# amazon-science/gan-control

Hardware: AMD Instinct MI355X
Metric: images/sec G+D step FFHQ-1024 (higher is better)
Workload: dtype bf16x3; 1 GPU; FFHQ 1024x1024 full G+D train step (D step, G step, lazy R1 every 16 and path-length every 4, Adam, EMA), 4 images/GPU, fp32 storage, conv arithmetic bf16x3; global_batch=4, parallelism=dp1

## Files before the change

### gan-control_amd/csrc/bias_act.hip

```cpp
#include "common.h"

namespace {

__device__ __forceinline__ float lrelu_gain(float v, float slope, float gain) {
    return (v > 0.f ? v : v * slope) * gain;
}

template <bool VEC, bool NOISE>
__global__ __launch_bounds__(256) void bias_act_plane_kernel(
    const float* __restrict__ x, const float* __restrict__ bias, const float* __restrict__ noise,
    const float* __restrict__ noise_w, float* __restrict__ y, int channels, int64_t inner, float slope, float gain) {
    const int plane = blockIdx.y;
    const int c = plane % channels, b = plane / channels;
    const float bv = bias ? bias[c] : 0.f;
    const float nw = NOISE ? noise_w[0] : 0.f;
    const float* xp = x + (size_t)plane * inner;
    float* yp = y + (size_t)plane * inner;
    const float* np = NOISE ? noise + (size_t)b * inner : nullptr;
    if (VEC) {
        const int64_t n4 = inner >> 2;
        for (int64_t i = (int64_t)blockIdx.x * 256 + threadIdx.x; i < n4; i += (int64_t)gridDim.x * 256) {
            const gc::f32x4_t xv = gc::stream_load4(xp + 4 * i);
            float4 v = make_float4(xv.x, xv.y, xv.z, xv.w);
            if (NOISE) {
                const float4 nz = reinterpret_cast<const float4*>(np)[i];
                v.x = fmaf(nw, nz.x, v.x); v.y = fmaf(nw, nz.y, v.y); v.z = fmaf(nw, nz.z, v.z); v.w = fmaf(nw, nz.w, v.w);
            }
            v.x = lrelu_gain(v.x + bv, slope, gain); v.y = lrelu_gain(v.y + bv, slope, gain);
            v.z = lrelu_gain(v.z + bv, slope, gain); v.w = lrelu_gain(v.w + bv, slope, gain);
            gc::stream_store4(yp + 4 * i, v.x, v.y, v.z, v.w);
        }
    } else {
        for (int64_t i = (int64_t)blockIdx.x * 256 + threadIdx.x; i < inner; i += (int64_t)gridDim.x * 256) {
            float v = xp[i];
            if (NOISE) v = fmaf(nw, np[i], v);
            yp[i] = lrelu_gain(v + bv, slope, gain);
        }
    }
}

template <bool NOISE>
__global__ __launch_bounds__(256) void bias_act_flat_kernel(
    const float* __restrict__ x, const float* __restrict__ bias, const float* __restrict__ noise,
    const float* __restrict__ noise_w, float* __restrict__ y, int channels, int inner, int64_t total, float slope, float gain) {
    const float nw = NOISE ? noise_w[0] : 0.f;
    for (int64_t i = (int64_t)blockIdx.x * 256 + threadIdx.x; i < total; i += (int64_t)gridDim.x * 256) {
        const int64_t plane = i / inner;
        const int p = (int)(i - plane * inner);
        const int c = (int)(plane % channels);
        float v = x[i];
        if (NOISE) v = fmaf(nw, noise[(plane / channels) * inner + p], v);
        y[i] = lrelu_gain(v + (bias ? bias[c] : 0.f), slope, gain);
    }
}

#ifndef GC_BWD_RUN
#define GC_BWD_RUN 1024
#endif
constexpr int BWD_RUN = GC_BWD_RUN;
template <bool VEC>
__global__ __launch_bounds__(256) void bias_act_bwd_kernel(
    const float* __restrict__ dy, const float* __restrict__ yref, float* __restrict__ dx, int64_t count, float pos, float neg) {
    if (VEC) {
        const int64_t n4 = count >> 2;
        const int64_t lo = (int64_t)blockIdx.x * BWD_RUN, hi = min(n4, lo + BWD_RUN);
        for (int64_t i = lo + threadIdx.x; i < hi; i += 256) {
            const gc::f32x4_t g = gc::stream_load4(dy + 4 * i);
            const gc::f32x4_t r = gc::stream_load4(yref + 4 * i);
            float4 o;
            o.x = g.x * (r.x > 0.f ? pos : neg); o.y = g.y * (r.y > 0.f ? pos : neg);
            o.z = g.z * (r.z > 0.f ? pos : neg); o.w = g.w * (r.w > 0.f ? pos : neg);
            gc::stream_store4(dx + 4 * i, o.x, o.y, o.z, o.w);
        }
        if (blockIdx.x == 0)
            for (int64_t i = (n4 << 2) + threadIdx.x; i < count; i += 256) dx[i] = dy[i] * (yref[i] > 0.f ? pos : neg);
    } else {
        const int64_t lo = (int64_t)blockIdx.x * (4 * BWD_RUN), hi = min(count, lo + 4 * BWD_RUN);
        for (int64_t i = lo + threadIdx.x; i < hi; i += 256) dx[i] = dy[i] * (yref[i] > 0.f ? pos : neg);
    }
}

__device__ __forceinline__ float wave_sum(float v) {
#pragma unroll
    for (int off = 32; off > 0; off >>= 1) v += __shfl_down(v, off, 64);
    return v;
}

__device__ __forceinline__ float block_sum(float v, float* lds) {
    v = wave_sum(v);
    const int lane = threadIdx.x & 63, wave = threadIdx.x >> 6;
    if (lane == 0) lds[wave] = v;
    __syncthreads();
    float r = 0.f;
    if (threadIdx.x == 0) r = lds[0] + lds[1] + lds[2] + lds[3];
    __syncthreads();
    return r;
}

template <bool NOISE, bool SELF>
__global__ __launch_bounds__(256) void bias_act_bwd_reduce_kernel(
    const float* __restrict__ dy, const float* __restrict__ yref, const float* __restrict__ noise, const float* __restrict__ bias,
    const float* __restrict__ noise_w, float* __restrict__ dx, float* __restrict__ psum, float* __restrict__ pdot, float* __restrict__ pself,
    int channels, int64_t inner, int chunks, int64_t chunk_len, float pos, float neg) {
    __shared__ float lds[4];
    const int plane = blockIdx.x / chunks, j = blockIdx.x - plane * chunks;
    const int b = plane / channels, c = plane % channels;
    const size_t base = (size_t)plane * inner;
    const float* np = NOISE ? noise + (size_t)b * inner : nullptr;
    const float bv = (SELF && bias) ? bias[c] : 0.f, nw = (SELF && NOISE) ? noise_w[0] : 0.f;
    const float ipos = 1.f / pos, ineg = 1.f / neg;
    const int64_t lo = (int64_t)j * chunk_len, hi = min(inner, lo + chunk_len);
    float s = 0.f, d = 0.f, q = 0.f;
    auto one = [&](float yv, float dyv, float nz) {
        const float g = dyv * (yv > 0.f ? pos : neg);
        s += g;
        if (NOISE) d = fmaf(g, nz, d);
        if (SELF) q = fmaf(g, yv * (yv > 0.f ? ipos : ineg) - bv - nw * nz, q);
        return g;
    };
    typedef float f4u __attribute__((ext_vector_type(4), aligned(4)));
    const int64_t n4 = (hi - lo) >> 2;
    for (int64_t v = threadIdx.x; v < n4; v += 256) {
        const int64_t i = lo + 4 * v;
        const f4u y4 = gc::stream_load4u(yref + base + i), g4 = gc::stream_load4u(dy + base + i);
        f4u z4 = {0.f, 0.f, 0.f, 0.f};
        if (NOISE) z4 = *reinterpret_cast<const f4u*>(np + i);
        const f4u o4 = {one(y4.x, g4.x, z4.x), one(y4.y, g4.y, z4.y), one(y4.z, g4.z, z4.z), one(y4.w, g4.w, z4.w)};
        gc::stream_store4u(dx + base + i, o4.x, o4.y, o4.z, o4.w);
    }
    for (int64_t i = lo + 4 * n4 + threadIdx.x; i < hi; i += 256)
        dx[base + i] = one(yref[base + i], dy[base + i], NOISE ? np[i] : 0.f);
    const float rs = block_sum(s, lds);
    if (threadIdx.x == 0) psum[(size_t)plane * chunks + j] = rs;
    if (NOISE) {
        const float rd = block_sum(d, lds);
        if (threadIdx.x == 0) pdot[(size_t)plane * chunks + j] = rd;
    }
    if (SELF) {
        const float rq = block_sum(q, lds);
        if (threadIdx.x == 0) pself[(size_t)plane * chunks + j] = rq;
    }
}

__global__ __launch_bounds__(256) void bias_act_bwd_reduce_adjoint_kernel(
    const float* __restrict__ ggx, const float* __restrict__ cs, const float* __restrict__ cd, const float* __restrict__ cw,
    const float* __restrict__ yref, const float* __restrict__ dx, const float* __restrict__ noise, const float* __restrict__ bias,
    const float* __restrict__ noise_w, float* __restrict__ g_dy, float* __restrict__ g_yref, float* __restrict__ pgb, float* __restrict__ pgn,
    int channels, int64_t inner, int chunks, int64_t chunk_len, float pos, float neg) {
    __shared__ float lds[4];
    const int plane = blockIdx.x / chunks, j = blockIdx.x - plane * chunks;
    const int b = plane / channels, c = plane % channels;
    const size_t base = (size_t)plane * inner, pj = (size_t)plane * chunks + j;
    const float* np = noise ? noise + (size_t)b * inner : nullptr;
    const float bv = bias ? bias[c] : 0.f, nw = (noise && noise_w) ? noise_w[0] : 0.f;
    const float ipos = 1.f / pos, ineg = 1.f / neg;
    const float vs = cs ? cs[pj] : 0.f, vd = (cd && noise) ? cd[pj] : 0.f, vw = cw ? cw[pj] : 0.f;
    const int64_t lo = (int64_t)j * chunk_len, hi = min(inner, lo + chunk_len);
    float sb = 0.f, sn = 0.f;
    typedef float f4u __attribute__((ext_vector_type(4), aligned(4)));
    auto one = [&](float yv, float gg, float gxv, float nz, float* gyref) {
        const bool up = yv > 0.f;
        const float xpre = yv * (up ? ipos : ineg) - bv - nw * nz;
        const float total = gg + vs + vd * nz + vw * xpre;
        const float wg = vw * gxv;
        sb += wg;
        sn = fmaf(wg, nz, sn);
        *gyref = wg * (up ? ipos : ineg);
        return total * (up ? pos : neg);
    };
    const int64_t n4 = (hi - lo) >> 2;
    for (int64_t v = threadIdx.x; v < n4; v += 256) {
        const int64_t i = lo + 4 * v;
        const f4u y4 = *reinterpret_cast<const f4u*>(yref + base + i);
        f4u g4 = {0.f, 0.f, 0.f, 0.f}, x4 = g4, z4 = g4;
        if (ggx) g4 = *reinterpret_cast<const f4u*>(ggx + base + i);
        if (cw) x4 = *reinterpret_cast<const f4u*>(dx + base + i);
        if (np) z4 = *reinterpret_cast<const f4u*>(np + i);
        float r0, r1, r2, r3;
        const f4u o4 = {one(y4.x, g4.x, x4.x, z4.x, &r0), one(y4.y, g4.y, x4.y, z4.y, &r1), one(y4.z, g4.z, x4.z, z4.z, &r2), one(y4.w, g4.w, x4.w, z4.w, &r3)};
        gc::stream_store4u(g_dy + base + i, o4.x, o4.y, o4.z, o4.w);
        if (g_yref) gc::stream_store4u(g_yref + base + i, r0, r1, r2, r3);
    }
    for (int64_t i = lo + 4 * n4 + threadIdx.x; i < hi; i += 256) {
        float r;
        g_dy[base + i] = one(yref[base + i], ggx ? ggx[base + i] : 0.f, cw ? dx[base + i] : 0.f, np ? np[i] : 0.f, &r);
        if (g_yref) g_yref[base + i] = r;
    }
    if (pgb) {
        const float rb = block_sum(sb, lds);
        if (threadIdx.x == 0) pgb[pj] = rb;
    }
    if (pgn) {
        const float rn = block_sum(sn, lds);
        if (threadIdx.x == 0) pgn[pj] = rn;
    }
}

__global__ __launch_bounds__(256) void plane_dot_kernel(const float* __restrict__ a, const float* __restrict__ b, float* __restrict__ partial,
                                                        int64_t inner, int chunks, int64_t chunk_len) {
    __shared__ float lds[4];
    const int plane = blockIdx.x / chunks, j = blockIdx.x - plane * chunks;
    const size_t base = (size_t)plane * inner;
    const int64_t lo = (int64_t)j * chunk_len, hi = min(inner, lo + chunk_len);
    float acc = 0.f;
    typedef float f4u __attribute__((ext_vector_type(4), aligned(4)));
    const int64_t n4 = (hi - lo) >> 2;
    for (int64_t v = threadIdx.x; v < n4; v += 256) {
        const int64_t i = lo + 4 * v;
        const f4u a4 = gc::stream_load4u(a + base + i), b4 = gc::stream_load4u(b + base + i);
        acc = fmaf(a4.x, b4.x, acc); acc = fmaf(a4.y, b4.y, acc); acc = fmaf(a4.z, b4.z, acc); acc = fmaf(a4.w, b4.w, acc);
    }
    for (int64_t i = lo + 4 * n4 + threadIdx.x; i < hi; i += 256) acc = fmaf(a[base + i], b[base + i], acc);
    const float r = block_sum(acc, lds);
    if (threadIdx.x == 0) partial[(size_t)plane * chunks + j] = r;
}

__global__ __launch_bounds__(256) void rows_sum_div_kernel(const float* __restrict__ partial, const float* __restrict__ den, float* __restrict__ out,
                                                           int rows, int chunks) {
    const int r = blockIdx.x * 256 + threadIdx.x;
    if (r >= rows) return;
    float acc = 0.f;
    for (int j = 0; j < chunks; ++j) acc += partial[(size_t)r * chunks + j];
    if (den) { const float d = den[r]; acc = acc / (d == 0.f ? 1.f : d); }
    out[r] = acc;
}

__global__ __launch_bounds__(256) void plane_dot_pitched_kernel(const float* __restrict__ a, const float* __restrict__ b, float* __restrict__ partial,
                                                                int rows, int width, int a_pitch, int b_pitch, int chunks, int rpc) {
    __shared__ float lds[4];
    const int plane = blockIdx.x / chunks, j = blockIdx.x - plane * chunks;
    const float* ap = a + (size_t)plane * rows * a_pitch;
    const float* bp = b + (size_t)plane * rows * b_pitch;
    const int r0 = j * rpc, r1 = min(rows, r0 + rpc);
    typedef float f4u __attribute__((ext_vector_type(4), aligned(4)));
    const int lane = threadIdx.x & 63, wave = threadIdx.x >> 6;
    const int w4 = width >> 2;
    float acc0 = 0.f, acc1 = 0.f;
    for (int r = r0 + wave; r < r1; r += 4) {
        const float* ar = ap + (size_t)r * a_pitch;
        const float* br = bp + (size_t)r * b_pitch;
        int v = lane;
        for (; v + 64 < w4; v += 128) {
            const f4u a0 = *reinterpret_cast<const f4u*>(ar + 4 * v), b0 = *reinterpret_cast<const f4u*>(br + 4 * v);
            const f4u a1 = *reinterpret_cast<const f4u*>(ar + 4 * (v + 64)), b1 = *reinterpret_cast<const f4u*>(br + 4 * (v + 64));
            acc0 = fmaf(a0.x, b0.x, acc0); acc0 = fmaf(a0.y, b0.y, acc0); acc0 = fmaf(a0.z, b0.z, acc0); acc0 = fmaf(a0.w, b0.w, acc0);
            acc1 = fmaf(a1.x, b1.x, acc1); acc1 = fmaf(a1.y, b1.y, acc1); acc1 = fmaf(a1.z, b1.z, acc1); acc1 = fmaf(a1.w, b1.w, acc1);
        }
        for (; v < w4; v += 64) {
            const f4u a0 = *reinterpret_cast<const f4u*>(ar + 4 * v), b0 = *reinterpret_cast<const f4u*>(br + 4 * v);
            acc0 = fmaf(a0.x, b0.x, acc0); acc0 = fmaf(a0.y, b0.y, acc0); acc0 = fmaf(a0.z, b0.z, acc0); acc0 = fmaf(a0.w, b0.w, acc0);
        }
        for (int c = 4 * w4 + lane; c < width; c += 64) acc1 = fmaf(ar[c], br[c], acc1);
    }
    const float s = block_sum(acc0 + acc1, lds);
    if (threadIdx.x == 0) partial[(size_t)plane * chunks + j] = s;
}

__global__ __launch_bounds__(256) void channel_sum_stage1(const float* __restrict__ x, float* __restrict__ partial,
                                                          int batch, int channels, int64_t inner, int chunks, int64_t chunk_len) {
    __shared__ float lds[4];
    const int plane = blockIdx.x / chunks, j = blockIdx.x - plane * chunks;
    const int c = plane % channels, b = plane / channels;
    const float* xp = x + (size_t)plane * inner;
    const int64_t lo = (int64_t)j * chunk_len, hi = min(inner, lo + chunk_len);
    float acc = 0.f;
    if (((inner | lo | hi) & 3) == 0 && (reinterpret_cast<uintptr_t>(xp) & 15) == 0) {
        const float4* x4 = reinterpret_cast<const float4*>(xp);
        float a0 = 0.f, a1 = 0.f, a2 = 0.f, a3 = 0.f;
#pragma unroll 4
        for (int64_t i = lo / 4 + threadIdx.x; i < hi / 4; i += 256) {
            const gc::f32x4_t v = gc::stream_load4(reinterpret_cast<const float*>(x4 + i));
            a0 += v.x; a1 += v.y; a2 += v.z; a3 += v.w;
        }
        acc = (a0 + a1) + (a2 + a3);
    } else {
        for (int64_t i = lo + threadIdx.x; i < hi; i += 256) acc += xp[i];
    }
    const float r = block_sum(acc, lds);
    if (threadIdx.x == 0) partial[((size_t)c * batch + b) * chunks + j] = r;
}

__global__ __launch_bounds__(256) void channel_sum_stage2(const float* __restrict__ partial, float* __restrict__ out, int n) {
    __shared__ float lds[4];
    const int c = blockIdx.x;
    float acc = 0.f;
    for (int i = threadIdx.x; i < n; i += 256) acc += partial[(size_t)c * n + i];
    const float r = block_sum(acc, lds);
    if (threadIdx.x == 0) out[c] = r;
}

inline void channel_sum_plan(int64_t inner, int* chunks, int64_t* chunk_len) {
#ifndef GC_SUM_LEN
#define GC_SUM_LEN 16384
#endif
    int64_t len = GC_SUM_LEN;
    int n = (int)gc::ceil_div64(inner, len);
    if (n < 1) n = 1;
    *chunks = n;
    *chunk_len = len;
}

inline bool aligned16(const void* p) { return (reinterpret_cast<uintptr_t>(p) & 15) == 0; }

}

extern "C" int gc_bias_act_f32(const float* x, const float* bias, const float* noise, const float* noise_w,
                               float* y, int batch, int channels, int64_t inner, float slope, float gain, gc_stream_t stream) {
    if (!x || !y) return gc::fail(GC_ERR_BAD_ARG, "gc_bias_act_f32: null pointer");
    if ((noise == nullptr) != (noise_w == nullptr)) return gc::fail(GC_ERR_BAD_ARG, "gc_bias_act_f32: noise and noise_w must both be set or both be null");
    if (batch < 0 || channels <= 0 || inner <= 0) return gc::fail(GC_ERR_BAD_ARG, "gc_bias_act_f32: bad extents");
    if (batch == 0) return GC_OK;
    hipStream_t s = (hipStream_t)stream;
    const int64_t planes = (int64_t)batch * channels;
    if (inner >= 1024 && planes <= 65535) {
        const bool vec = (inner % 4 == 0) && aligned16(x) && aligned16(y) && (!noise || aligned16(noise));
        const int64_t work = vec ? inner / 4 : inner;
        dim3 grid((unsigned)std::min<int64_t>(gc::ceil_div64(work, 256 * 4), 1024), (unsigned)planes);
#define GC_LAUNCH(V, N) hipLaunchKernelGGL((bias_act_plane_kernel<V, N>), grid, dim3(256), 0, s, x, bias, noise, noise_w, y, channels, inner, slope, gain)
        if (vec) { if (noise) GC_LAUNCH(true, true); else GC_LAUNCH(true, false); }
        else     { if (noise) GC_LAUNCH(false, true); else GC_LAUNCH(false, false); }
#undef GC_LAUNCH
        return gc::check_launch("gc_bias_act_f32(plane)");
    }
    if (inner > INT32_MAX) return gc::fail(GC_ERR_UNSUPPORTED, "gc_bias_act_f32: inner too large for the flat path");
    const int64_t total = planes * inner;
    const int blocks = (int)std::min<int64_t>(gc::ceil_div64(total, 256), 4096);
    if (noise)
        hipLaunchKernelGGL(bias_act_flat_kernel<true>, dim3(blocks), dim3(256), 0, s, x, bias, noise, noise_w, y, channels, (int)inner, total, slope, gain);
    else
        hipLaunchKernelGGL(bias_act_flat_kernel<false>, dim3(blocks), dim3(256), 0, s, x, bias, noise, noise_w, y, channels, (int)inner, total, slope, gain);
    return gc::check_launch("gc_bias_act_f32(flat)");
}

extern "C" int gc_bias_act_bwd_f32(const float* dy, const float* y_ref, float* dx, int64_t count,
                                   float slope, float gain, gc_stream_t stream) {
    if (!dy || !y_ref || !dx) return gc::fail(GC_ERR_BAD_ARG, "gc_bias_act_bwd_f32: null pointer");
    if (count < 0) return gc::fail(GC_ERR_BAD_ARG, "gc_bias_act_bwd_f32: negative count");
    if (count == 0) return GC_OK;
    hipStream_t s = (hipStream_t)stream;
    const bool vec = aligned16(dy) && aligned16(y_ref) && aligned16(dx);
    const int64_t nblocks = gc::ceil_div64(count, 4 * (int64_t)BWD_RUN);
    if (nblocks > INT32_MAX) return gc::fail(GC_ERR_UNSUPPORTED, "gc_bias_act_bwd_f32: more than 2^31 blocks");
    const int blocks = (int)nblocks;
    if (vec)
        hipLaunchKernelGGL(bias_act_bwd_kernel<true>, dim3(blocks), dim3(256), 0, s, dy, y_ref, dx, count, gain, gain * slope);
    else
        hipLaunchKernelGGL(bias_act_bwd_kernel<false>, dim3(blocks), dim3(256), 0, s, dy, y_ref, dx, count, gain, gain * slope);
    return gc::check_launch("gc_bias_act_bwd_f32");
}

extern "C" size_t gc_channel_sum_workspace(int batch, int channels, int64_t inner) {
    if (batch <= 0 || channels <= 0 || inner <= 0) return 0;
    int chunks; int64_t len;
    channel_sum_plan(inner, &chunks, &len);
    return (size_t)batch * channels * chunks * sizeof(float);
}

extern "C" int gc_channel_sum_f32(const float* x, float* out, int batch, int channels, int64_t inner,
                                  void* workspace, size_t workspace_bytes, gc_stream_t stream) {
    if (!x || !out) return gc::fail(GC_ERR_BAD_ARG, "gc_channel_sum_f32: null pointer");
    if (batch <= 0 || channels <= 0 || inner <= 0) return gc::fail(GC_ERR_BAD_ARG, "gc_channel_sum_f32: bad extents");
    if ((int64_t)batch * channels * gc_bias_act_bwd_chunks(inner) > INT32_MAX) return gc::fail(GC_ERR_UNSUPPORTED, "gc_channel_sum_f32: more than 2^31 blocks");
    const size_t need = gc_channel_sum_workspace(batch, channels, inner);
    if (!workspace || workspace_bytes < need) return gc::fail(GC_ERR_WORKSPACE, "gc_channel_sum_f32: workspace %zu < %zu bytes", workspace_bytes, need);
    hipStream_t s = (hipStream_t)stream;
    int chunks; int64_t len;
    channel_sum_plan(inner, &chunks, &len);
    float* partial = static_cast<float*>(workspace);
    hipLaunchKernelGGL(channel_sum_stage1, dim3((unsigned)chunks * (unsigned)(batch * channels)), dim3(256), 0, s, x, partial, batch, channels, inner, chunks, len);
    int rc = gc::check_launch("gc_channel_sum_f32(stage1)");
    if (rc) return rc;
    hipLaunchKernelGGL(channel_sum_stage2, dim3(channels), dim3(256), 0, s, partial, out, batch * chunks);
    return gc::check_launch("gc_channel_sum_f32(stage2)");
}

extern "C" int gc_bias_act_bwd_chunks(int64_t inner) {
    if (inner <= 0) return 0;
    int chunks; int64_t len;
    channel_sum_plan(inner, &chunks, &len);
    return chunks;
}

extern "C" int gc_bias_act_bwd_reduce_self_f32(const float* dy, const float* y_ref, const float* noise, const float* bias, const float* noise_w,
                                               float* dx, float* psum, float* pdot, float* pself, int batch, int channels, int64_t inner,
                                               float slope, float gain, gc_stream_t stream) {
    if (!dy || !y_ref || !dx || !psum) return gc::fail(GC_ERR_BAD_ARG, "gc_bias_act_bwd_reduce_f32: null pointer");
    if ((noise == nullptr) != (pdot == nullptr)) return gc::fail(GC_ERR_BAD_ARG, "gc_bias_act_bwd_reduce_f32: noise and pdot go together");
    if (pself && noise && !noise_w) return gc::fail(GC_ERR_BAD_ARG, "gc_bias_act_bwd_reduce_f32: pself with noise needs noise_w");
    if (pself && (slope == 0.f || gain == 0.f)) return gc::fail(GC_ERR_UNSUPPORTED, "gc_bias_act_bwd_reduce_f32: pself needs an invertible activation (slope, gain != 0)");
    if (batch <= 0 || channels <= 0 || inner <= 0) return gc::fail(GC_ERR_BAD_ARG, "gc_bias_act_bwd_reduce_f32: bad extents");
    hipStream_t s = (hipStream_t)stream;
    int chunks; int64_t len;
    channel_sum_plan(inner, &chunks, &len);
    if ((int64_t)batch * channels * chunks > INT32_MAX) return gc::fail(GC_ERR_UNSUPPORTED, "gc_bias_act_bwd_reduce_f32: more than 2^31 blocks");
    dim3 grid((unsigned)chunks * (unsigned)(batch * channels));
#define GC_LAUNCH(N, S) hipLaunchKernelGGL((bias_act_bwd_reduce_kernel<N, S>), grid, dim3(256), 0, s, dy, y_ref, noise, bias, noise_w, dx, psum, pdot, pself, \
                                           channels, inner, chunks, len, gain, gain * slope)
    if (noise) { if (pself) GC_LAUNCH(true, true); else GC_LAUNCH(true, false); }
    else       { if (pself) GC_LAUNCH(false, true); else GC_LAUNCH(false, false); }
#undef GC_LAUNCH
    return gc::check_launch("gc_bias_act_bwd_reduce_f32");
}

extern "C" int gc_bias_act_bwd_reduce_adjoint_f32(const float* ggx, const float* cs, const float* cd, const float* cw, const float* y_ref, const float* dx,
                                                  const float* noise, const float* bias, const float* noise_w, float* g_dy, float* g_yref, float* pgb, float* pgn,
                                                  int batch, int channels, int64_t inner, float slope, float gain, gc_stream_t stream) {
    if (!y_ref || !g_dy) return gc::fail(GC_ERR_BAD_ARG, "gc_bias_act_bwd_reduce_adjoint_f32: null pointer");
    if (cw && !dx) return gc::fail(GC_ERR_BAD_ARG, "gc_bias_act_bwd_reduce_adjoint_f32: cw needs dx");
    if (cw && noise && !noise_w) return gc::fail(GC_ERR_BAD_ARG, "gc_bias_act_bwd_reduce_adjoint_f32: cw with noise needs noise_w");
    if (cd && !noise) return gc::fail(GC_ERR_BAD_ARG, "gc_bias_act_bwd_reduce_adjoint_f32: cd needs noise");
    if (slope == 0.f || gain == 0.f) return gc::fail(GC_ERR_UNSUPPORTED, "gc_bias_act_bwd_reduce_adjoint_f32: needs an invertible activation (slope, gain != 0)");
    if (batch <= 0 || channels <= 0 || inner <= 0) return gc::fail(GC_ERR_BAD_ARG, "gc_bias_act_bwd_reduce_adjoint_f32: bad extents");
    int chunks; int64_t len;
    channel_sum_plan(inner, &chunks, &len);
    if ((int64_t)batch * channels * chunks > INT32_MAX) return gc::fail(GC_ERR_UNSUPPORTED, "gc_bias_act_bwd_reduce_adjoint_f32: more than 2^31 blocks");
    hipLaunchKernelGGL(bias_act_bwd_reduce_adjoint_kernel, dim3((unsigned)chunks * (unsigned)(batch * channels)), dim3(256), 0, (hipStream_t)stream, ggx, cs, cd, cw, y_ref, dx,
                       noise, bias, noise_w, g_dy, g_yref, pgb, pgn, channels, inner, chunks, len, gain, gain * slope);
    return gc::check_launch("gc_bias_act_bwd_reduce_adjoint_f32");
}

extern "C" int gc_bias_act_bwd_reduce_f32(const float* dy, const float* y_ref, const float* noise, float* dx,
                                          float* psum, float* pdot, int batch, int channels, int64_t inner,
                                          float slope, float gain, gc_stream_t stream) {
    return gc_bias_act_bwd_reduce_self_f32(dy, y_ref, noise, nullptr, nullptr, dx, psum, pdot, nullptr, batch, channels, inner, slope, gain, stream);
}

static void plane_dot_pitched_plan(int rows, int* chunks, int* rpc) {
    *rpc = rows <= 64 ? rows : 32;
    *chunks = (rows + *rpc - 1) / *rpc;
}

extern "C" int gc_plane_dot_pitched_chunks(int rows) {
    if (rows <= 0) return 0;
    int chunks, rpc;
    plane_dot_pitched_plan(rows, &chunks, &rpc);
    return chunks;
}

extern "C" int gc_plane_dot_pitched_f32(const float* a, const float* b, float* partial, int planes, int rows, int width, int a_pitch, int b_pitch,
                                        gc_stream_t stream) {
    if (!a || !b || !partial) return gc::fail(GC_ERR_BAD_ARG, "gc_plane_dot_pitched_f32: null pointer");
    if (planes <= 0 || rows <= 0 || width <= 0 || a_pitch < width || b_pitch < width) return gc::fail(GC_ERR_BAD_ARG, "gc_plane_dot_pitched_f32: bad extents");
    int chunks, rpc;
    plane_dot_pitched_plan(rows, &chunks, &rpc);
    if ((int64_t)planes * chunks > INT32_MAX) return gc::fail(GC_ERR_UNSUPPORTED, "gc_plane_dot_pitched_f32: more than 2^31 blocks");
    hipLaunchKernelGGL(plane_dot_pitched_kernel, dim3((unsigned)planes * (unsigned)chunks), dim3(256), 0, (hipStream_t)stream,
                       a, b, partial, rows, width, a_pitch, b_pitch, chunks, rpc);
    return gc::check_launch("gc_plane_dot_pitched_f32");
}

extern "C" int gc_rows_sum_div_f32(const float* partial, const float* den, float* out, int rows, int chunks, gc_stream_t stream) {
    if (!partial || !out) return gc::fail(GC_ERR_BAD_ARG, "gc_rows_sum_div_f32: null pointer");
    if (rows <= 0 || chunks <= 0) return gc::fail(GC_ERR_BAD_ARG, "gc_rows_sum_div_f32: bad extents");
    hipLaunchKernelGGL(rows_sum_div_kernel, dim3((unsigned)((rows + 255) / 256)), dim3(256), 0, (hipStream_t)stream, partial, den, out, rows, chunks);
    return gc::check_launch("gc_rows_sum_div_f32");
}

extern "C" int gc_plane_dot_f32(const float* a, const float* b, float* partial, int planes, int64_t inner, gc_stream_t stream) {
    if (!a || !b || !partial) return gc::fail(GC_ERR_BAD_ARG, "gc_plane_dot_f32: null pointer");
    if (planes <= 0 || inner <= 0) return gc::fail(GC_ERR_BAD_ARG, "gc_plane_dot_f32: bad extents");
    int chunks; int64_t len;
    channel_sum_plan(inner, &chunks, &len);
    if ((int64_t)planes * chunks > INT32_MAX) return gc::fail(GC_ERR_UNSUPPORTED, "gc_plane_dot_f32: more than 2^31 blocks");
    hipLaunchKernelGGL(plane_dot_kernel, dim3((unsigned)chunks * (unsigned)planes), dim3(256), 0, (hipStream_t)stream, a, b, partial, inner, chunks, len);
    return gc::check_launch("gc_plane_dot_f32");
}
```

### gan-control_amd/csrc/upfirdn2d.hip

```cpp
#include "common.h"

namespace {

constexpr int TH = 32, TW = 128;
constexpr int PH = TH + 3, PW = TW + 3;
constexpr int PITCH = 132;

struct FirEpilogue {
    const float* bias; const float* noise; const float* noise_w;
    float slope, gain; int channels;
    const float* mask_ref; float mpos, mneg;
    const float* pro_ref; const float* pro_noise; float* pro_psum; float* pro_pdot; float ppos, pneg;
};

#ifndef GC_FIR_NT
#define GC_FIR_NT 1
#endif

#ifndef GC_FIR_OCC
#define GC_FIR_OCC 0
#endif
#if GC_FIR_OCC > 0
#define GC_FIR_BOUNDS __launch_bounds__(256, GC_FIR_OCC)
#else
#define GC_FIR_BOUNDS __launch_bounds__(256)
#endif
template <bool VEC, int EPI, bool PRO = false>
__global__ GC_FIR_BOUNDS void fir44_tile_kernel(
    const float* __restrict__ x, const float* __restrict__ taps, float* __restrict__ y,
    int in_h, int in_w, int out_h, int out_w, int pad_x0, int pad_y0, int flip, FirEpilogue ep, int in_pitch, int out_pitch) {
    __shared__ __attribute__((aligned(16))) float patch[PH * PITCH];
    const int tid = threadIdx.x;
    const int ox0 = blockIdx.x * TW;
    const size_t plane = blockIdx.z;
    const float* xp = x + plane * (size_t)in_h * in_pitch;
    float* yp = y + plane * (size_t)out_h * out_pitch;

    float T[4][4];
#pragma unroll
    for (int a = 0; a < 4; ++a)
#pragma unroll
        for (int b = 0; b < 4; ++b) T[a][b] = flip ? taps[(3 - a) * 4 + (3 - b)] : taps[a * 4 + b];

    const int ix0 = ox0 - pad_x0;
    constexpr int GPR = PITCH / 4;
    constexpr int NLD = (PH * GPR + 255) / 256;
    typedef float f4u __attribute__((ext_vector_type(4), aligned(4)));
    float4 stage[NLD];
    auto ld4 = [&](const float* rowp, int ix, int width) {
        float4 v = make_float4(0.f, 0.f, 0.f, 0.f);
        const float* src = rowp + ix;
        if (ix >= 0 && ix + 3 < width) {
            const f4u t = *reinterpret_cast<const f4u*>(src);
            v = make_float4(t.x, t.y, t.z, t.w);
        } else {
            if (ix >= 0 && ix < width) v.x = src[0];
            if (ix + 1 >= 0 && ix + 1 < width) v.y = src[1];
            if (ix + 2 >= 0 && ix + 2 < width) v.z = src[2];
            if (ix + 3 >= 0 && ix + 3 < width) v.w = src[3];
        }
        return v;
    };
    static_assert(!PRO || GC_FIR_NT == 1, "the prologue sums are written once per workgroup");
    float ps = 0.f, pd = 0.f;
    const float* refp = PRO ? ep.pro_ref + plane * (size_t)in_h * in_w : nullptr;
    const float* nzp = (PRO && ep.pro_noise) ? ep.pro_noise + (plane / ep.channels) * (size_t)in_h * in_w : nullptr;
    auto fetch = [&](int oy0) {
        const int iy0 = oy0 - pad_y0;
#pragma unroll
        for (int j = 0; j < NLD; ++j) {
            const int idx = tid + 256 * j;
            const int r = idx / GPR, c = (idx - r * GPR) * 4;
            const int iy = iy0 + r, ix = ix0 + c;
            float4 v = make_float4(0.f, 0.f, 0.f, 0.f);
            if (idx < PH * GPR && iy >= 0 && iy < in_h) {
                v = ld4(xp + (size_t)iy * in_pitch, ix, in_w);
                if (PRO) {
                    const float4 m = ld4(refp + (size_t)iy * in_w, ix, in_w);
                    v.x *= m.x > 0.f ? ep.ppos : ep.pneg; v.y *= m.y > 0.f ? ep.ppos : ep.pneg;
                    v.z *= m.z > 0.f ? ep.ppos : ep.pneg; v.w *= m.w > 0.f ? ep.ppos : ep.pneg;
                    if ((r < TH || blockIdx.y == gridDim.y - 1) && (c < TW || blockIdx.x == gridDim.x - 1)) {
                        ps += (v.x + v.y) + (v.z + v.w);
                        if (nzp) {
                            const float4 z = ld4(nzp + (size_t)iy * in_w, ix, in_w);
                            pd += (v.x * z.x + v.y * z.y) + (v.z * z.z + v.w * z.w);
                        }
                    }
                }
            }
            stage[j] = v;
        }
    };
    auto commit = [&]() {
#pragma unroll
        for (int j = 0; j < NLD; ++j) {
            const int idx = tid + 256 * j;
            if (idx < PH * GPR) *reinterpret_cast<float4*>(&patch[idx * 4]) = stage[j];
        }
    };

    const int cg = tid & 31, rg = tid >> 5;
    const int ox = ox0 + cg * 4;
    const int ty0 = blockIdx.y * GC_FIR_NT;
    const int tiles_y = (out_h + TH - 1) / TH;
    const int nt = min(GC_FIR_NT, tiles_y - ty0);
    fetch(ty0 * TH);
    __shared__ float red[8];
    if (PRO) {
#pragma unroll
        for (int off = 32; off > 0; off >>= 1) { ps += __shfl_xor(ps, off, 64); pd += __shfl_xor(pd, off, 64); }
        if ((tid & 63) == 0) { red[(tid >> 6) * 2] = ps; red[(tid >> 6) * 2 + 1] = pd; }
    }
    commit();
    __syncthreads();
    if (PRO && tid == 0) {
        const size_t slot = plane * ((size_t)gridDim.x * gridDim.y) + (size_t)blockIdx.y * gridDim.x + blockIdx.x;
        ep.pro_psum[slot] = (red[0] + red[2]) + (red[4] + red[6]);
        if (ep.pro_pdot) ep.pro_pdot[slot] = (red[1] + red[3]) + (red[5] + red[7]);
    }
    for (int t = 0; t < nt; ++t) {
        const int oy0 = (ty0 + t) * TH;
        const bool more = t + 1 < nt;
        if (more) fetch(oy0 + TH);

        float acc[4][4];
#pragma unroll
        for (int r = 0; r < 4; ++r)
#pragma unroll
            for (int j = 0; j < 4; ++j) acc[r][j] = 0.f;

#pragma unroll
        for (int i = 0; i < 7; ++i) {
            const float* row = &patch[(rg * 4 + i) * PITCH + cg * 4];
            const float4 lo = *reinterpret_cast<const float4*>(row);
            const float v4 = row[4], v5 = row[5], v6 = row[6];
            const float v[7] = {lo.x, lo.y, lo.z, lo.w, v4, v5, v6};
#pragma unroll
            for (int r = 0; r < 4; ++r) {
                const int a = i - r;
                if (a < 0 || a > 3) continue;
#pragma unroll
                for (int j = 0; j < 4; ++j)
#pragma unroll
                    for (int b = 0; b < 4; ++b) acc[r][j] = fmaf(T[a][b], v[j + b], acc[r][j]);
            }
        }

        if (EPI == 2) {
            const float* ref = ep.mask_ref + plane * (size_t)out_h * out_w;
            float m[4][4];
            const bool vec_ref = VEC && (out_w & 3) == 0 && ((reinterpret_cast<uintptr_t>(ref) & 15) == 0);
#pragma unroll
            for (int r = 0; r < 4; ++r) {
                const int oy = oy0 + rg * 4 + r;
                if (vec_ref && oy < out_h && ox + 3 < out_w) {
                    const float4 t = *reinterpret_cast<const float4*>(ref + (size_t)oy * out_w + ox);
                    m[r][0] = t.x; m[r][1] = t.y; m[r][2] = t.z; m[r][3] = t.w;
                } else {
#pragma unroll
                    for (int j = 0; j < 4; ++j) m[r][j] = (oy < out_h && ox + j < out_w) ? ref[(size_t)oy * out_w + ox + j] : 0.f;
                }
            }
#pragma unroll
            for (int r = 0; r < 4; ++r)
#pragma unroll
                for (int j = 0; j < 4; ++j) acc[r][j] *= m[r][j] > 0.f ? ep.mpos : ep.mneg;
        }
        if (EPI == 1) {
            const int c = (int)(plane % ep.channels);
            const size_t b = plane / ep.channels;
            const float bv = ep.bias ? ep.bias[c] : 0.f, nw = ep.noise ? ep.noise_w[0] : 0.f;
            float nz[4][4];
#pragma unroll
            for (int r = 0; r < 4; ++r)
#pragma unroll
                for (int j = 0; j < 4; ++j) {
                    const int oy = oy0 + rg * 4 + r;
                    nz[r][j] = (ep.noise && oy < out_h && ox + j < out_w) ? ep.noise[(b * out_h + oy) * out_w + ox + j] : 0.f;
                }
#pragma unroll
            for (int r = 0; r < 4; ++r)
#pragma unroll
                for (int j = 0; j < 4; ++j) {
                    const float v = fmaf(nw, nz[r][j], acc[r][j]) + bv;
                    acc[r][j] = (v > 0.f ? v : v * ep.slope) * ep.gain;
                }
        }
        if (more) {
            __syncthreads();
            commit();
            __syncthreads();
        }
#pragma unroll
        for (int r = 0; r < 4; ++r) {
            const int oy = oy0 + rg * 4 + r;
            if (oy >= out_h) break;
            float* dst = yp + (size_t)oy * out_pitch + ox;
            if (VEC) {
                if (ox + 3 < out_w) gc::stream_store4(dst, acc[r][0], acc[r][1], acc[r][2], acc[r][3]);
                else {
#pragma unroll
                    for (int j = 0; j < 4; ++j)
                        if (ox + j < out_w) dst[j] = acc[r][j];
                }
            } else if (ox + 3 < out_w) {
                gc::stream_store4u(dst, acc[r][0], acc[r][1], acc[r][2], acc[r][3]);
            } else {
#pragma unroll
                for (int j = 0; j < 4; ++j)
                    if (ox + j < out_w) dst[j] = acc[r][j];
            }
        }
    }
}


constexpr int D_TH = 16, D_TW = 128;
constexpr int D_PH = 2 * D_TH + 2, D_PW = 2 * D_TW + 2, D_PITCH = 260;

template <bool VEC>
__global__ __launch_bounds__(256) void fir44_down2_kernel(
    const float* __restrict__ x, const float* __restrict__ taps, float* __restrict__ y,
    int in_h, int in_w, int out_h, int out_w, int pad_x0, int pad_y0, int flip) {
    __shared__ __attribute__((aligned(16))) float patch[D_PH * D_PITCH];
    const int tid = threadIdx.x;
    const int ox0 = blockIdx.x * D_TW, oy0 = blockIdx.y * D_TH;
    const size_t plane = blockIdx.z;
    const float* xp = x + plane * (size_t)in_h * in_w;
    float* yp = y + plane * (size_t)out_h * out_w;

    float T[4][4];
#pragma unroll
    for (int a = 0; a < 4; ++a)
#pragma unroll
        for (int b = 0; b < 4; ++b) T[a][b] = flip ? taps[(3 - a) * 4 + (3 - b)] : taps[a * 4 + b];

    const int iy0 = 2 * oy0 - pad_y0, ix0 = 2 * ox0 - pad_x0;
    constexpr int GPR = D_PITCH / 4;
    constexpr int NLD = (D_PH * GPR + 255) / 256;
    typedef float f4u __attribute__((ext_vector_type(4), aligned(4)));
    float4 stage[NLD];
#pragma unroll
    for (int j = 0; j < NLD; ++j) {
        const int idx = tid + 256 * j;
        const int r = idx / GPR, c = (idx - r * GPR) * 4;
        const int iy = iy0 + r, ix = ix0 + c;
        float4 v = make_float4(0.f, 0.f, 0.f, 0.f);
        if (idx < D_PH * GPR && iy >= 0 && iy < in_h) {
            const float* src = xp + (size_t)iy * in_w + ix;
            if (ix >= 0 && ix + 3 < in_w) {
                const f4u t = *reinterpret_cast<const f4u*>(src);
                v = make_float4(t.x, t.y, t.z, t.w);
            } else {
                if (ix >= 0 && ix < in_w) v.x = src[0];
                if (ix + 1 >= 0 && ix + 1 < in_w) v.y = src[1];
                if (ix + 2 >= 0 && ix + 2 < in_w) v.z = src[2];
                if (ix + 3 >= 0 && ix + 3 < in_w) v.w = src[3];
            }
        }
        stage[j] = v;
    }
#pragma unroll
    for (int j = 0; j < NLD; ++j) {
        const int idx = tid + 256 * j;
        if (idx < D_PH * GPR) *reinterpret_cast<float4*>(&patch[idx * 4]) = stage[j];
    }
    __syncthreads();

    const int cg = tid & 31, rg = tid >> 5;
    float acc[2][4];
#pragma unroll
    for (int r = 0; r < 2; ++r)
#pragma unroll
        for (int j = 0; j < 4; ++j) acc[r][j] = 0.f;
#pragma unroll
    for (int i = 0; i < 6; ++i) {
        const float* row = &patch[(rg * 4 + i) * D_PITCH + cg * 8];
        const float4 q0 = *reinterpret_cast<const float4*>(row), q1 = *reinterpret_cast<const float4*>(row + 4);
        const float2 q2 = *reinterpret_cast<const float2*>(row + 8);
        const float v[10] = {q0.x, q0.y, q0.z, q0.w, q1.x, q1.y, q1.z, q1.w, q2.x, q2.y};
#pragma unroll
        for (int r = 0; r < 2; ++r) {
            const int a = i - 2 * r;
            if (a < 0 || a > 3) continue;
#pragma unroll
            for (int j = 0; j < 4; ++j)
#pragma unroll
                for (int b = 0; b < 4; ++b) acc[r][j] = fmaf(T[a][b], v[2 * j + b], acc[r][j]);
        }
    }
    const int ox = ox0 + cg * 4;
#pragma unroll
    for (int r = 0; r < 2; ++r) {
        const int oy = oy0 + rg * 2 + r;
        if (oy >= out_h) break;
        float* dst = yp + (size_t)oy * out_w + ox;
        if (VEC) {
            if (ox + 3 < out_w) gc::stream_store4(dst, acc[r][0], acc[r][1], acc[r][2], acc[r][3]);
        } else if (ox + 3 < out_w) {
            gc::stream_store4u(dst, acc[r][0], acc[r][1], acc[r][2], acc[r][3]);
        } else {
#pragma unroll
            for (int j = 0; j < 4; ++j)
                if (ox + j < out_w) dst[j] = acc[r][j];
        }
    }
}

constexpr int U_TH = 32, U_TW = 128;
constexpr int U_PH = U_TH / 2 + 3, U_PW = U_TW / 2 + 3, U_PITCH = 68;

template <int EY, int EX, bool VEC>
__global__ __launch_bounds__(256) void fir44_up2_kernel(
    const float* __restrict__ x, const float* __restrict__ taps, float* __restrict__ y,
    int in_h, int in_w, int out_h, int out_w, int pad_x0, int pad_y0, int flip) {
    __shared__ __attribute__((aligned(16))) float patch[U_PH * U_PITCH];
    const int tid = threadIdx.x;
    const int ox0 = blockIdx.x * U_TW, oy0 = blockIdx.y * U_TH;
    const size_t plane = blockIdx.z;
    const float* xp = x + plane * (size_t)in_h * in_w;
    float* yp = y + plane * (size_t)out_h * out_w;

    float T[4][4];
#pragma unroll
    for (int a = 0; a < 4; ++a)
#pragma unroll
        for (int b = 0; b < 4; ++b) T[a][b] = flip ? taps[(3 - a) * 4 + (3 - b)] : taps[a * 4 + b];

    const int iy0 = (oy0 - pad_y0) >> 1, ix0 = (ox0 - pad_x0) >> 1;
    constexpr int NLD = (U_PH * U_PITCH + 255) / 256;
    float stage[NLD];
#pragma unroll
    for (int j = 0; j < NLD; ++j) {
        const int idx = tid + 256 * j;
        const int r = idx / U_PITCH, c = idx - r * U_PITCH;
        const int iy = iy0 + r, ix = ix0 + c;
        float v = 0.f;
        if (idx < U_PH * U_PITCH && c < U_PW && iy >= 0 && iy < in_h && ix >= 0 && ix < in_w) v = xp[(size_t)iy * in_w + ix];
        stage[j] = v;
    }
#pragma unroll
    for (int j = 0; j < NLD; ++j) {
        const int idx = tid + 256 * j;
        if (idx < U_PH * U_PITCH) patch[idx] = stage[j];
    }
    __syncthreads();

    const int cg = tid & 31, rg = tid >> 5;
    float w[4][4];
#pragma unroll
    for (int i = 0; i < 4; ++i) {
        const float* row = &patch[(rg * 2 + i) * U_PITCH + cg * 2];
        const float2 lo = *reinterpret_cast<const float2*>(row), hi = *reinterpret_cast<const float2*>(row + 2);
        w[i][0] = lo.x; w[i][1] = lo.y; w[i][2] = hi.x; w[i][3] = hi.y;
    }
    const int ox = ox0 + cg * 4;
#pragma unroll
    for (int r = 0; r < 4; ++r) {
        const int a0 = (EY + r) & 1, qy = (EY + r + a0) >> 1;
        float o[4];
#pragma unroll
        for (int j = 0; j < 4; ++j) {
            const int b0 = (EX + j) & 1, qx = (EX + j + b0) >> 1;
            float s = 0.f;
#pragma unroll
            for (int i = 0; i < 2; ++i)
#pragma unroll
                for (int jj = 0; jj < 2; ++jj) s = fmaf(T[a0 + 2 * i][b0 + 2 * jj], w[qy + i][qx + jj], s);
            o[j] = s;
        }
        const int oy = oy0 + rg * 4 + r;
        if (oy < out_h) {
            float* dst = yp + (size_t)oy * out_w + ox;
            if (VEC) {
                if (ox + 3 < out_w) gc::stream_store4(dst, o[0], o[1], o[2], o[3]);
            } else if (ox + 3 < out_w) {
                gc::stream_store4u(dst, o[0], o[1], o[2], o[3]);
            } else {
#pragma unroll
                for (int j = 0; j < 4; ++j)
                    if (ox + j < out_w) dst[j] = o[j];
            }
        }
    }
}

constexpr int SMALL_LDS_FLOATS = 4096, SMALL_PLANE_MAX = 36 * 36;

__global__ __launch_bounds__(256) void fir44_small_kernel(
    const float* __restrict__ x, const float* __restrict__ taps, float* __restrict__ y,
    int planes, int in_h, int in_w, int out_h, int out_w, int pad_x0, int pad_y0, int flip, int ppw) {
    __shared__ float L[SMALL_LDS_FLOATS];
    __shared__ float T[16];
    const int tid = threadIdx.x;
    if (tid < 16) T[tid] = flip ? taps[15 - tid] : taps[tid];
    const int lh = out_h + 3, lw = out_w + 3, lp = lh * lw;
    const int p0 = blockIdx.x * ppw, np = min(ppw, planes - p0);
    const float* xb = x + (size_t)p0 * in_h * in_w;
    for (int i = tid; i < np * lp; i += 256) {
        const int pl = i / lp, rem = i - pl * lp;
        const int r = rem / lw, c = rem - r * lw;
        const int iy = r - pad_y0, ix = c - pad_x0;
        L[i] = (iy >= 0 && iy < in_h && ix >= 0 && ix < in_w) ? xb[((size_t)pl * in_h + iy) * in_w + ix] : 0.f;
    }
    __syncthreads();
    const int op = out_h * out_w;
    float* yb = y + (size_t)p0 * op;
    for (int i = tid; i < np * op; i += 256) {
        const int pl = i / op, rem = i - pl * op;
        const int oy = rem / out_w, ox = rem - oy * out_w;
        const float* l = L + pl * lp + oy * lw + ox;
        float acc = 0.f;
#pragma unroll
        for (int a = 0; a < 4; ++a)
#pragma unroll
            for (int b = 0; b < 4; ++b) acc = fmaf(T[a * 4 + b], l[a * lw + b], acc);
        yb[i] = acc;
    }
}

constexpr int MAX_GENERIC_TAPS = 1024;

__global__ __launch_bounds__(256) void generic_kernel(
    const float* __restrict__ x, const float* __restrict__ taps, float* __restrict__ y,
    int planes, int in_h, int in_w, int out_h, int out_w, int kh, int kw,
    int up_x, int up_y, int down_x, int down_y, int pad_x0, int pad_y0, int flip) {
    __shared__ float T[MAX_GENERIC_TAPS];
    const int nt = kh * kw;
    for (int i = threadIdx.x; i < nt; i += 256) T[i] = flip ? taps[nt - 1 - i] : taps[i];
    __syncthreads();
    const size_t total = (size_t)planes * out_h * out_w;
    for (size_t idx = (size_t)blockIdx.x * 256 + threadIdx.x; idx < total; idx += (size_t)gridDim.x * 256) {
        const int ox = (int)(idx % out_w);
        const size_t t = idx / out_w;
        const int oy = (int)(t % out_h);
        const size_t plane = t / out_h;
        const float* xp = x + plane * (size_t)in_h * in_w;
        const int uy0 = oy * down_y - pad_y0, ux0 = ox * down_x - pad_x0;
        const int a0 = gc::pos_mod(-uy0, up_y), b0 = gc::pos_mod(-ux0, up_x);
        float acc = 0.f;
        for (int a = a0; a < kh; a += up_y) {
            const int uy = uy0 + a;
            if (uy < 0) continue;
            const int iy = uy / up_y;
            if (iy >= in_h) break;
            for (int b = b0; b < kw; b += up_x) {
                const int ux = ux0 + b;
                if (ux < 0) continue;
                const int ix = ux / up_x;
                if (ix >= in_w) break;
                acc = fmaf(T[a * kw + b], xp[(size_t)iy * in_w + ix], acc);
            }
        }
        y[idx] = acc;
    }
}

template <int K, int UP, int DOWN>
struct FirKCfg {
    static constexpr int TW = 64, TH = 16;
    static constexpr int PW = ((TW - 1) * DOWN + K - 1) / UP + 2, PH = ((TH - 1) * DOWN + K - 1) / UP + 2;
    static constexpr int PITCH = PW | 1;
};

template <int K, int UP, int DOWN>
__global__ __launch_bounds__(256) void firK_tile_kernel(
    const float* __restrict__ x, const float* __restrict__ taps, float* __restrict__ y,
    int in_h, int in_w, int out_h, int out_w, int pad_x0, int pad_y0, int flip) {
    using C = FirKCfg<K, UP, DOWN>;
    __shared__ float patch[C::PH * C::PITCH];
    __shared__ float T[K * K];
    const int tid = threadIdx.x;
    const int ox0 = blockIdx.x * C::TW, oy0 = blockIdx.y * C::TH;
    const size_t plane = blockIdx.z;
    const float* xp = x + plane * (size_t)in_h * in_w;
    float* yp = y + plane * (size_t)out_h * out_w;
    for (int i = tid; i < K * K; i += 256) T[i] = flip ? taps[K * K - 1 - i] : taps[i];
    const int ux_base = ox0 * DOWN - pad_x0, uy_base = oy0 * DOWN - pad_y0;
    const int ixb = gc::floor_div(ux_base, UP), iyb = gc::floor_div(uy_base, UP);
    for (int i = tid; i < C::PH * C::PW; i += 256) {
        const int r = i / C::PW, c = i - r * C::PW;
        const int iy = iyb + r, ix = ixb + c;
        patch[r * C::PITCH + c] = (iy >= 0 && iy < in_h && ix >= 0 && ix < in_w) ? xp[(size_t)iy * in_w + ix] : 0.f;
    }
    __syncthreads();
    const int ty = tid >> 4, tx = (tid & 15) * 4;
    const int oy = oy0 + ty;
    if (oy >= out_h) return;
    const int uy0 = oy * DOWN - pad_y0;
    const int a0 = gc::pos_mod(-uy0, UP);
    float acc[4] = {0.f, 0.f, 0.f, 0.f};
    int b0[4], cx[4];
#pragma unroll
    for (int i = 0; i < 4; ++i) {
        const int ux0 = (ox0 + tx + i) * DOWN - pad_x0;
        b0[i] = gc::pos_mod(-ux0, UP);
        cx[i] = (ux0 + b0[i] - ixb * UP) / UP;
    }
    constexpr int NA = (K + UP - 1) / UP;
#pragma unroll 2
    for (int aa = 0; aa < NA; ++aa) {
        const int a = a0 + aa * UP;
        if (a >= K) break;
        const float* prow = patch + ((uy0 + a - iyb * UP) / UP) * C::PITCH;
        const float* trow = T + a * K;
#pragma unroll
        for (int bb = 0; bb < NA; ++bb) {
#pragma unroll
            for (int i = 0; i < 4; ++i) {
                const int b = b0[i] + bb * UP;
                if (UP == 1 || b < K) acc[i] = fmaf(trow[b], prow[cx[i] + bb], acc[i]);
            }
        }
    }
#pragma unroll
    for (int i = 0; i < 4; ++i)
        if (ox0 + tx + i < out_w) yp[(size_t)oy * out_w + ox0 + tx + i] = acc[i];
}

template <int K>
int launch_firK(const float* x, const float* taps, float* y, int planes, int in_h, int in_w, int out_h, int out_w,
                int up, int down, int pad_x0, int pad_y0, int flip, hipStream_t s) {
    using C = FirKCfg<K, 1, 1>;
    dim3 grid(gc::ceil_div(out_w, C::TW), gc::ceil_div(out_h, C::TH), planes);
    if (up == 2 && down == 1)
        hipLaunchKernelGGL((firK_tile_kernel<K, 2, 1>), grid, dim3(256), 0, s, x, taps, y, in_h, in_w, out_h, out_w, pad_x0, pad_y0, flip);
    else if (up == 1 && down == 2)
        hipLaunchKernelGGL((firK_tile_kernel<K, 1, 2>), grid, dim3(256), 0, s, x, taps, y, in_h, in_w, out_h, out_w, pad_x0, pad_y0, flip);
    else
        hipLaunchKernelGGL((firK_tile_kernel<K, 1, 1>), grid, dim3(256), 0, s, x, taps, y, in_h, in_w, out_h, out_w, pad_x0, pad_y0, flip);
    return gc::check_launch("gc_upfirdn2d_f32(firK_tile)");
}

}

namespace {

int upfirdn2d_impl(const float* x, const float* taps, float* y,
                   int planes, int in_h, int in_w, int out_h, int out_w,
                   int kh, int kw, int up_x, int up_y, int down_x, int down_y,
                   int pad_x0, int pad_y0, int flip_taps, const FirEpilogue* ep, gc_stream_t stream, int in_pitch = 0, int out_pitch = 0) {
    if (in_pitch == 0) in_pitch = in_w;
    if (out_pitch == 0) out_pitch = out_w;
    if (out_pitch < out_w) return gc::fail(GC_ERR_BAD_ARG, "gc_upfirdn2d_f32: output pitch %d < width %d", out_pitch, out_w);
    if (in_pitch < in_w) return gc::fail(GC_ERR_BAD_ARG, "gc_upfirdn2d_f32: input pitch %d < width %d", in_pitch, in_w);
    if (!x || !taps || !y) return gc::fail(GC_ERR_BAD_ARG, "gc_upfirdn2d_f32: null pointer");
    if (planes < 0 || in_h <= 0 || in_w <= 0 || kh <= 0 || kw <= 0 || up_x <= 0 || up_y <= 0 || down_x <= 0 || down_y <= 0)
        return gc::fail(GC_ERR_BAD_ARG, "gc_upfirdn2d_f32: non-positive extent or factor");
    if (out_h <= 0 || out_w <= 0) return gc::fail(GC_ERR_BAD_ARG, "gc_upfirdn2d_f32: empty output (%d x %d)", out_h, out_w);
    if (planes == 0) return GC_OK;
    hipStream_t s = (hipStream_t)stream;
    const bool fast = up_x == 1 && up_y == 1 && down_x == 1 && down_y == 1 && kh == 4 && kw == 4 &&
                      out_w >= 64 && out_h >= 16 && planes <= 65535;
    if (ep && !fast) return gc::fail(GC_ERR_UNSUPPORTED, "gc_upfirdn2d_act_f32: the fused epilogue needs the 4x4, up = down = 1 tile kernel (planes >= 64 x 16)");
    if ((in_pitch != in_w || out_pitch != out_w) && !fast) return gc::fail(GC_ERR_UNSUPPORTED, "gc_upfirdn2d_pitched_f32: a pitched input needs the 4x4, up = down = 1 tile kernel (planes >= 64 x 16)");
    if (fast) {
        dim3 grid(gc::ceil_div(out_w, TW), gc::ceil_div(gc::ceil_div(out_h, TH), GC_FIR_NT), planes);
        const bool vec = (out_pitch % 4 == 0) && ((reinterpret_cast<uintptr_t>(y) & 15) == 0);
        const FirEpilogue none{nullptr, nullptr, nullptr, 1.f, 1.f, 1, nullptr, 1.f, 1.f, nullptr, nullptr, nullptr, nullptr, 1.f, 1.f};
        if (ep && ep->pro_ref) {
            if (in_pitch != in_w) return gc::fail(GC_ERR_UNSUPPORTED, "gc_upfirdn2d_actbwd_f32: the gradient must have dense rows");
            if (vec) hipLaunchKernelGGL((fir44_tile_kernel<true, 0, true>), grid, dim3(256), 0, s, x, taps, y, in_h, in_w, out_h, out_w, pad_x0, pad_y0, flip_taps, *ep, in_pitch, out_pitch);
            else     hipLaunchKernelGGL((fir44_tile_kernel<false, 0, true>), grid, dim3(256), 0, s, x, taps, y, in_h, in_w, out_h, out_w, pad_x0, pad_y0, flip_taps, *ep, in_pitch, out_pitch);
            return gc::check_launch("gc_upfirdn2d_actbwd_f32");
        }
#define GC_FIR(V, E) hipLaunchKernelGGL((fir44_tile_kernel<V, E>), grid, dim3(256), 0, s, x, taps, y, in_h, in_w, out_h, out_w, pad_x0, pad_y0, flip_taps, ep ? *ep : none, in_pitch, out_pitch)
        if (ep && ep->mask_ref) { if (vec) GC_FIR(true, 2); else GC_FIR(false, 2); }
        else if (ep) { if (vec) GC_FIR(true, 1); else GC_FIR(false, 1); }
        else    { if (vec) GC_FIR(true, 0); else GC_FIR(false, 0); }
#undef GC_FIR
        return gc::check_launch("gc_upfirdn2d_f32(fir44_tile)");
    }
    if (kh == 4 && kw == 4 && up_x == 1 && up_y == 1 && down_x == 1 && down_y == 1 && (out_h + 3) * (out_w + 3) <= SMALL_PLANE_MAX) {
        const int ppw = std::max(1, std::min(SMALL_LDS_FLOATS / ((out_h + 3) * (out_w + 3)), 1024 / std::max(1, out_h * out_w) + 1));
        hipLaunchKernelGGL(fir44_small_kernel, dim3(gc::ceil_div(planes, ppw)), dim3(256), 0, s, x, taps, y, planes, in_h, in_w, out_h, out_w,
                           pad_x0, pad_y0, flip_taps, ppw);
        return gc::check_launch("gc_upfirdn2d_f32(fir44_small)");
    }
    const bool square44 = kh == 4 && kw == 4 && up_x == up_y && down_x == down_y && planes <= 65535 && out_w >= 32 && out_h >= 8;
    const bool vec_ok = (out_w % 4 == 0) && ((reinterpret_cast<uintptr_t>(y) & 15) == 0);
    if (square44 && up_x == 1 && down_x == 2) {
        dim3 grid(gc::ceil_div(out_w, D_TW), gc::ceil_div(out_h, D_TH), planes);
        if (vec_ok)
            hipLaunchKernelGGL(fir44_down2_kernel<true>, grid, dim3(256), 0, s, x, taps, y, in_h, in_w, out_h, out_w, pad_x0, pad_y0, flip_taps);
        else
            hipLaunchKernelGGL(fir44_down2_kernel<false>, grid, dim3(256), 0, s, x, taps, y, in_h, in_w, out_h, out_w, pad_x0, pad_y0, flip_taps);
        return gc::check_launch("gc_upfirdn2d_f32(fir44_down2)");
    }
    if (square44 && up_x == 2 && down_x == 1) {
        dim3 grid(gc::ceil_div(out_w, U_TW), gc::ceil_div(out_h, U_TH), planes);
        const int ey = pad_y0 & 1, ex = pad_x0 & 1;
#define GC_UP2(EY, EX)                                                                                                             \
        if (ey == EY && ex == EX) {                                                                                                \
            if (vec_ok) hipLaunchKernelGGL((fir44_up2_kernel<EY, EX, true>), grid, dim3(256), 0, s, x, taps, y, in_h, in_w, out_h, out_w, pad_x0, pad_y0, flip_taps); \
            else hipLaunchKernelGGL((fir44_up2_kernel<EY, EX, false>), grid, dim3(256), 0, s, x, taps, y, in_h, in_w, out_h, out_w, pad_x0, pad_y0, flip_taps);       \
        }
        GC_UP2(0, 0) GC_UP2(0, 1) GC_UP2(1, 0) GC_UP2(1, 1)
#undef GC_UP2
        return gc::check_launch("gc_upfirdn2d_f32(fir44_up2)");
    }
    if (kh == 12 && kw == 12 && up_x == up_y && down_x == down_y && up_x * down_x <= 2 && planes <= 65535 && out_w >= 32 && out_h >= 8)
        return launch_firK<12>(x, taps, y, planes, in_h, in_w, out_h, out_w, up_x, down_x, pad_x0, pad_y0, flip_taps, s);
    if (kh * kw > MAX_GENERIC_TAPS) return gc::fail(GC_ERR_UNSUPPORTED, "gc_upfirdn2d_f32: %d x %d taps exceed %d", kh, kw, MAX_GENERIC_TAPS);
    const size_t total = (size_t)planes * out_h * out_w;
    const int blocks = (int)std::min<size_t>((total + 255) / 256, 256 * 16);
    hipLaunchKernelGGL(generic_kernel, dim3(blocks), dim3(256), 0, s, x, taps, y, planes, in_h, in_w, out_h, out_w, kh, kw,
                       up_x, up_y, down_x, down_y, pad_x0, pad_y0, flip_taps);
    return gc::check_launch("gc_upfirdn2d_f32(generic)");
}

}

extern "C" int gc_upfirdn2d_f32(const float* x, const float* taps, float* y,
                                int planes, int in_h, int in_w, int out_h, int out_w,
                                int kh, int kw, int up_x, int up_y, int down_x, int down_y,
                                int pad_x0, int pad_y0, int flip_taps, gc_stream_t stream) {
    return upfirdn2d_impl(x, taps, y, planes, in_h, in_w, out_h, out_w, kh, kw, up_x, up_y, down_x, down_y, pad_x0, pad_y0, flip_taps, nullptr, stream);
}

extern "C" int gc_upfirdn2d_pitched_f32(const float* x, const float* taps, float* y, int batch, int channels, int in_h, int in_w, int in_pitch,
                                        int out_h, int out_w, int out_pitch, int kh, int kw, int pad_x0, int pad_y0, int flip_taps, int activate,
                                        const float* bias, const float* noise, const float* noise_w, float slope, float gain, gc_stream_t stream) {
    if ((noise == nullptr) != (noise_w == nullptr)) return gc::fail(GC_ERR_BAD_ARG, "gc_upfirdn2d_pitched_f32: noise and noise_w must both be set or both be null");
    if (batch < 0 || channels <= 0) return gc::fail(GC_ERR_BAD_ARG, "gc_upfirdn2d_pitched_f32: bad batch / channels");
    const bool epi = activate || bias || noise;
    const FirEpilogue ep{bias, noise, noise_w, activate ? slope : 1.f, activate ? gain : 1.f, channels, nullptr, 1.f, 1.f, nullptr, nullptr, nullptr, nullptr, 1.f, 1.f};
    return upfirdn2d_impl(x, taps, y, batch * channels, in_h, in_w, out_h, out_w, kh, kw, 1, 1, 1, 1, pad_x0, pad_y0, flip_taps, epi ? &ep : nullptr, stream, in_pitch, out_pitch);
}

extern "C" int gc_upfirdn2d_actbwd_tiles(int out_h, int out_w) {
    if (out_h <= 0 || out_w <= 0) return 0;
    return gc::ceil_div(out_w, TW) * gc::ceil_div(gc::ceil_div(out_h, TH), GC_FIR_NT);
}

extern "C" int gc_upfirdn2d_actbwd_f32(const float* gy, const float* y_ref, const float* noise, const float* taps, float* gx, float* psum, float* pdot,
                                       int batch, int channels, int in_h, int in_w, int out_h, int out_w, int out_pitch, int kh, int kw,
                                       int pad_x0, int pad_y0, int flip_taps, float slope, float gain, gc_stream_t stream) {
    if (!y_ref || !psum) return gc::fail(GC_ERR_BAD_ARG, "gc_upfirdn2d_actbwd_f32: null pointer");
    if ((noise == nullptr) != (pdot == nullptr)) return gc::fail(GC_ERR_BAD_ARG, "gc_upfirdn2d_actbwd_f32: noise and pdot go together");
    if (batch < 0 || channels <= 0) return gc::fail(GC_ERR_BAD_ARG, "gc_upfirdn2d_actbwd_f32: bad batch / channels");
    const FirEpilogue ep{nullptr, nullptr, nullptr, 1.f, 1.f, channels, nullptr, 1.f, 1.f, y_ref, noise, psum, pdot, gain, gain * slope};
    return upfirdn2d_impl(gy, taps, gx, batch * channels, in_h, in_w, out_h, out_w, kh, kw, 1, 1, 1, 1, pad_x0, pad_y0, flip_taps, &ep, stream, 0, out_pitch);
}

extern "C" int gc_upfirdn2d_mask_f32(const float* x, const float* taps, float* y, int batch, int channels, int in_h, int in_w, int in_pitch,
                                     int out_h, int out_w, int kh, int kw, int pad_x0, int pad_y0, int flip_taps,
                                     const float* mask_ref, float slope, float gain, gc_stream_t stream) {
    if (!mask_ref) return gc::fail(GC_ERR_BAD_ARG, "gc_upfirdn2d_mask_f32: null mask reference");
    if (batch < 0 || channels <= 0) return gc::fail(GC_ERR_BAD_ARG, "gc_upfirdn2d_mask_f32: bad batch / channels");
    const FirEpilogue ep{nullptr, nullptr, nullptr, 1.f, 1.f, channels, mask_ref, gain, gain * slope, nullptr, nullptr, nullptr, nullptr, 1.f, 1.f};
    return upfirdn2d_impl(x, taps, y, batch * channels, in_h, in_w, out_h, out_w, kh, kw, 1, 1, 1, 1, pad_x0, pad_y0, flip_taps, &ep, stream, in_pitch, 0);
}

extern "C" int gc_upfirdn2d_act_f32(const float* x, const float* taps, float* y,
                                    int batch, int channels, int in_h, int in_w, int out_h, int out_w,
                                    int kh, int kw, int pad_x0, int pad_y0, int flip_taps,
                                    const float* bias, const float* noise, const float* noise_w, float slope, float gain,
                                    gc_stream_t stream) {
    if ((noise == nullptr) != (noise_w == nullptr)) return gc::fail(GC_ERR_BAD_ARG, "gc_upfirdn2d_act_f32: noise and noise_w must both be set or both be null");
    if (batch < 0 || channels <= 0) return gc::fail(GC_ERR_BAD_ARG, "gc_upfirdn2d_act_f32: bad batch / channels");
    const FirEpilogue ep{bias, noise, noise_w, slope, gain, channels, nullptr, 1.f, 1.f, nullptr, nullptr, nullptr, nullptr, 1.f, 1.f};
    return upfirdn2d_impl(x, taps, y, batch * channels, in_h, in_w, out_h, out_w, kh, kw, 1, 1, 1, 1, pad_x0, pad_y0, flip_taps, &ep, stream);
}
```

### gan-control_amd/gan_control_amd/_lib.py

```python
import ctypes
import os

import torch

_HERE = os.path.dirname(os.path.abspath(__file__))
_DEFAULT = os.path.normpath(os.path.join(_HERE, '..', 'csrc', 'libgancontrol_hip.so'))

ABI_VERSION = 2
MODE_IDS = {'f32': 0, 'bf16x3': 1, 'bf16': 2}

_i32, _i64, _f32, _vp, _sz = ctypes.c_int32, ctypes.c_int64, ctypes.c_float, ctypes.c_void_p, ctypes.c_size_t


class ConvDesc(ctypes.Structure):
    _fields_ = [(n, _i32) for n in ('batch', 'in_ch', 'out_ch', 'in_h', 'in_w', 'out_h', 'out_w',
                                    'kh', 'kw', 'up', 'down', 'pad_y', 'pad_x', 'in_pitch', 'out_pitch')]


class ConvEpilogue(ctypes.Structure):
    _fields_ = [('bias', _vp), ('noise', _vp), ('noise_w', _vp), ('slope', _f32), ('gain', _f32), ('activate', _i32), ('residual', _vp)]


class GlinGroup(ctypes.Structure):
    _fields_ = [('x', _vp), ('w', _vp), ('bias', _vp), ('y', _vp), ('n', _i32), ('k', _i32), ('x_stride', _i64), ('alpha', _f32), ('beta', _f32)]


class WLayoutGroup(ctypes.Structure):
    _fields_ = [('src', _vp), ('dst', _vp), ('taps', _i32), ('k', _i32), ('n', _i32), ('flip_taps', _i32), ('src_stride', _i64 * 3), ('dst_stride', _i64 * 3), ('scale', _f32)]


class WPackGroup(ctypes.Structure):
    _fields_ = [('desc', ConvDesc), ('w', _vp), ('packed', _vp), ('packed_bytes', _sz)]


class WsqGroup(ctypes.Structure):
    _fields_ = [('w', _vp), ('g', _vp), ('out', _vp), ('rows', _i32), ('taps', _i32)]


STRUCTS = (ConvDesc, ConvEpilogue, WLayoutGroup, WPackGroup, GlinGroup, WsqGroup)

SIGNATURES = {
    'gc_abi_version': (_i32, []),
    'gc_last_error': (ctypes.c_char_p, []),
    'gc_struct_sizes': (_i32, [ctypes.POINTER(_sz), _i32]),
    'gc_source_hash': (ctypes.c_char_p, []),
    'gc_upfirdn2d_f32': (_i32, [_vp, _vp, _vp] + [_i32] * 14 + [_vp]),
    'gc_upfirdn2d_act_f32': (_i32, [_vp, _vp, _vp] + [_i32] * 11 + [_vp, _vp, _vp, _f32, _f32, _vp]),
    'gc_bias_act_f32': (_i32, [_vp, _vp, _vp, _vp, _vp, _i32, _i32, _i64, _f32, _f32, _vp]),
    'gc_bias_act_bwd_f32': (_i32, [_vp, _vp, _vp, _i64, _f32, _f32, _vp]),
    'gc_bias_act_bwd_chunks': (_i32, [_i64]),
    'gc_bias_act_bwd_reduce_f32': (_i32, [_vp, _vp, _vp, _vp, _vp, _vp, _i32, _i32, _i64, _f32, _f32, _vp]),
    'gc_bias_act_bwd_reduce_self_f32': (_i32, [_vp, _vp, _vp, _vp, _vp, _vp, _vp, _vp, _vp, _i32, _i32, _i64, _f32, _f32, _vp]),
    'gc_bias_act_bwd_reduce_adjoint_f32': (_i32, [_vp] * 13 + [_i32, _i32, _i64, _f32, _f32, _vp]),
    'gc_plane_dot_f32': (_i32, [_vp, _vp, _vp, _i32, _i64, _vp]),
    'gc_rows_sum_div_f32': (_i32, [_vp, _vp, _vp, _i32, _i32, _vp]),
    'gc_conv2d_bn_relu_f32': (_i32, [_vp, _vp, _vp, _vp, _vp] + [_i32] * 13 + [_vp]),
    'gc_pool2d_f32': (_i32, [_vp, _vp] + [_i32] * 10 + [_vp]),
    'gc_global_avgpool_f32': (_i32, [_vp, _vp, _i32, _i32, _vp]),
    'gc_resize_bilinear_f32': (_i32, [_vp, _vp, _i32, _i32, _i32, _i32, _i32, _f32, _f32, _vp]),
    'gc_channel_sum_workspace': (_sz, [_i32, _i32, _i64]),
    'gc_channel_sum_f32': (_i32, [_vp, _vp, _i32, _i32, _i64, _vp, _sz, _vp]),
    'gc_conv2d_f32': (_i32, [ctypes.POINTER(ConvDesc), _vp, _vp, _vp, _vp, _vp, _vp]),
    'gc_conv2d_fused_f32': (_i32, [ctypes.POINTER(ConvDesc), _vp, _vp, _vp, _vp, ctypes.POINTER(ConvEpilogue), _vp, _vp]),
    'gc_conv2d_f32_workspace': (_sz, [ctypes.POINTER(ConvDesc)]),
    'gc_small_gemm_ok': (_i32, [_i32, _i32, _i32, _i64, _i64]),
    'gc_small_gemm_f32': (_i32, [_vp, _i64, _i64, _vp, _i64, _i64, _vp, _f32, _f32, _vp, _i32, _i32, _i32, _vp]),
    'gc_conv2d_fused_f32_ws': (_i32, [ctypes.POINTER(ConvDesc), _vp, _vp, _vp, _vp, ctypes.POINTER(ConvEpilogue), _vp, _vp, _sz, _vp]),
    'gc_conv2d_fused_bf16x3_f32': (_i32, [ctypes.POINTER(ConvDesc), _vp, _vp, _vp, _vp, ctypes.POINTER(ConvEpilogue), _vp, _vp, _sz, _vp]),
    'gc_conv2d_bf16x3_workspace': (_sz, [ctypes.POINTER(ConvDesc)]),
    'gc_conv2d_bf16x3_packed_bytes': (_sz, [ctypes.POINTER(ConvDesc)]),
    'gc_conv2d_bf16x3_splitk_bytes': (_sz, [ctypes.POINTER(ConvDesc)]),
    'gc_conv2d_pack_weights_bf16x3': (_i32, [ctypes.POINTER(ConvDesc), _vp, _vp, _sz, _vp]),
    'gc_conv2d_fused_bf16x3_packed_f32': (_i32, [ctypes.POINTER(ConvDesc), _vp, _vp, _vp, _sz, _vp, _vp, ctypes.POINTER(ConvEpilogue), _vp, _vp, _sz, _vp]),
    'gc_conv2d_fused_bf16_packed_f32': (_i32, [ctypes.POINTER(ConvDesc), _vp, _vp, _vp, _sz, _vp, _vp, ctypes.POINTER(ConvEpilogue), _vp, _vp, _sz, _vp]),
    'gc_conv2d_wgrad_bf16_f32': (_i32, [ctypes.POINTER(ConvDesc), _vp, _vp, _vp, _vp, _vp, _vp, _sz, _vp]),
    'gc_conv2d_variant_name': (_i32, [ctypes.POINTER(ConvDesc), _i32, ctypes.c_char_p, _i32]),
    'gc_conv2d_wgrad_variant_name': (_i32, [ctypes.POINTER(ConvDesc), _i32, _i32, ctypes.c_char_p, _i32]),
    'gc_conv2d_out_pitch': (_i32, [ctypes.POINTER(ConvDesc), _i32]),
    'gc_conv2d_in_pitch_ok': (_i32, [ctypes.POINTER(ConvDesc), _i32, _i32]),
    'gc_upfirdn2d_actbwd_tiles': (_i32, [_i32, _i32]),
    'gc_upfirdn2d_actbwd_f32': (_i32, [_vp] * 7 + [_i32] * 12 + [_f32, _f32, _vp]),
    'gc_upfirdn2d_mask_f32': (_i32, [_vp, _vp, _vp] + [_i32] * 12 + [_vp, _f32, _f32, _vp]),
    'gc_upfirdn2d_pitched_f32': (_i32, [_vp, _vp, _vp] + [_i32] * 14 + [_vp, _vp, _vp, _f32, _f32, _vp]),
    'gc_plane_dot_pitched_chunks': (_i32, [_i32]),
    'gc_plane_dot_pitched_f32': (_i32, [_vp, _vp, _vp, _i32, _i32, _i32, _i32, _i32, _vp]),
    'gc_conv2d_bf16x3_f32': (_i32, [ctypes.POINTER(ConvDesc), _vp, _vp, _vp, _vp, _vp, _vp, _sz, _vp]),
    'gc_conv2d_wgrad_workspace': (_sz, [ctypes.POINTER(ConvDesc)]),
    'gc_conv2d_wgrad_f32': (_i32, [ctypes.POINTER(ConvDesc), _vp, _vp, _vp, _vp, _vp, _vp, _sz, _vp]),
    'gc_conv2d_wgrad_bf16x3_workspace': (_sz, [ctypes.POINTER(ConvDesc)]),
    'gc_conv2d_wgrad_bf16x3_f32': (_i32, [ctypes.POINTER(ConvDesc), _vp, _vp, _vp, _vp, _vp, _vp, _sz, _vp]),
    'gc_conv2d_wgrad_samples_workspace': (_sz, [ctypes.POINTER(ConvDesc), _i32]),
    'gc_conv2d_wgrad_samples_f32': (_i32, [ctypes.POINTER(ConvDesc), _vp, _vp, _vp, _vp, _vp, _vp, _vp, _sz, _vp]),
    'gc_conv2d_wgrad_samples_bf16x3_f32': (_i32, [ctypes.POINTER(ConvDesc), _vp, _vp, _vp, _vp, _vp, _vp, _vp, _sz, _vp]),
    'gc_conv2d_wgrad_samples_bf16_f32': (_i32, [ctypes.POINTER(ConvDesc), _vp, _vp, _vp, _vp, _vp, _vp, _vp, _sz, _vp]),
    'gc_wgrad_samples_contract_workspace': (_sz, [_i32, _i32, _i32]),
    'gc_wgrad_samples_contract_f32': (_i32, [_vp, _vp, _vp, _vp, _vp, _vp, _i32, _i32, _i32, _i32, _vp, _sz, _vp]),
    'gc_affine_warp_bilinear_f32': (_i32, [_vp, _vp, _vp] + [_i32] * 7 + [_vp]),
    'gc_reflect_pad_f32': (_i32, [_vp, _vp] + [_i32] * 8 + [_vp]),
    'gc_pw_act_wgrad_workspace': (_sz, [_i32, _i32, _i32, _i64]),
    'gc_pw_act_wgrad_f32': (_i32, [_vp, _vp, _vp, _vp, _i32, _i32, _i32, _i64, _f32, _f32, _vp, _sz, _vp]),
    'gc_pw_act_dgrad_f32': (_i32, [_vp, _vp, _vp, _vp, _i32, _i32, _i32, _i64, _f32, _f32, _vp]),
    'gc_grouped_linear_f32': (_i32, [ctypes.POINTER(GlinGroup), _i32, _i32, _vp]),
    'gc_grouped_linear_bwd_x_f32': (_i32, [ctypes.POINTER(GlinGroup), _i32, _i32, _vp]),
    'gc_grouped_linear_bwd_w_f32': (_i32, [ctypes.POINTER(GlinGroup), _i32, _i32, _vp]),
    'gc_weight_sq_grouped_f32': (_i32, [ctypes.POINTER(WsqGroup), _i32, _vp]),
    'gc_weight_sq_bwd_grouped_f32': (_i32, [ctypes.POINTER(WsqGroup), _i32, _vp]),
    'gc_crop_resize_ac_f32': (_i32, [_vp, _vp] + [_i32] * 10 + [_vp]),
    'gc_affine_prelu_f32': (_i32, [_vp] * 5 + [_i32] * 3 + [_vp]),
    'gc_affine_prelu_bwd_f32': (_i32, [_vp] * 6 + [_i32, _vp] + [_i32] * 4 + [_vp]),
    'gc_plane_reduce_f32': (_i32, [_vp, _vp, _vp, _i32, _i32, _f32, _vp]),
    'gc_se_mlp_f32': (_i32, [_vp] * 5 + [_i32] * 3 + [_vp]),
    'gc_se_mlp_bwd_f32': (_i32, [_vp] * 6 + [_i32] * 3 + [_f32, _vp]),
    'gc_se_apply_f32': (_i32, [_vp] * 4 + [_i32] * 6 + [_vp]),
    'gc_weight_layout_grouped_f32': (_i32, [ctypes.POINTER(WLayoutGroup), _i32, _vp]),
    'gc_conv2d_pack_weights_bf16x3_grouped': (_i32, [ctypes.POINTER(WPackGroup), _i32, _vp]),
    'gc_image_u8_to_f32': (_i32, [_vp, _i64, _i64, _vp, _vp, _vp, _i32, _i32, _i32, _vp]),
    'gc_image_resample_u8': (_i32, [_vp, _i64, _i64, _i32, _i32, _vp, _i32, _i32, _i32, _i32, _vp, _vp, _vp, _i32, _i32, _vp, _vp, _vp]),
    'gc_image_resample_v_u8_to_f32': (_i32, [_vp, _i64, _i64, _i32, _i32, _vp, _vp, _vp, _i32, _i32, _i32, _vp, _vp, _vp, _i32, _i32, _vp, _vp, _vp]),
    'gc_image_f32_to_u8_grid': (_i32, [_vp, _i64, _i64, _i64, _vp, _i64] + [_i32] * 8 + [_vp]),
    'gc_weight_layout_f32': (_i32, [_vp, _vp, _i32, _i32, _i32, ctypes.POINTER(_i64 * 3), ctypes.POINTER(_i64 * 3), _i32, _f32, _vp]),
}

_lib = None


def source_hash():
    v = load().gc_source_hash()
    return v.decode() if v else None


def library_path():
    return os.environ.get('GANCONTROL_HIP_LIB', _DEFAULT)


def load():
    global _lib
    if _lib is not None:
        return _lib
    path = library_path()
    if not os.path.exists(path):
        raise RuntimeError(
            f'gan_control_amd: HIP kernel library not found at {path}. Build it with '
            f'`make -C gan-control_amd/csrc` (or `python -c "import __graft_entry__ as g; g.build()"`). '
            f'There is no CPU or PyTorch fallback for the hot path.')
    try:
        lib = ctypes.CDLL(path)
    except OSError as e:
        raise RuntimeError(f'gan_control_amd: cannot load {path}: {e}') from e
    for name, (res, args) in SIGNATURES.items():
        try:
            fn = getattr(lib, name)
        except AttributeError as e:
            raise RuntimeError(f'gan_control_amd: {path} does not export {name}') from e
        fn.restype, fn.argtypes = res, args
    if lib.gc_abi_version() != ABI_VERSION:
        raise RuntimeError(f'gan_control_amd: ABI version {lib.gc_abi_version()} != {ABI_VERSION}; rebuild the library')
    theirs = (_sz * len(STRUCTS))()
    count = lib.gc_struct_sizes(theirs, len(STRUCTS))
    ours = [ctypes.sizeof(c) for c in STRUCTS]
    if count != len(STRUCTS) or list(theirs) != ours:
        raise RuntimeError(f'gan_control_amd: {path} was built from another header: struct sizes {list(theirs)[:count]} (library) != {ours} '
                           f'(binding: {[c.__name__ for c in STRUCTS]}); rebuild the library')
    _lib = lib
    return lib


class UnsupportedError(RuntimeError):
    """GC_ERR_UNSUPPORTED: a legal request outside what the kernels implement -- the one failure a caller may answer with another route."""


GC_ERR_UNSUPPORTED = -2


def check(rc, what):
    if rc != 0:
        msg = load().gc_last_error()
        kind = UnsupportedError if rc == GC_ERR_UNSUPPORTED else RuntimeError
        raise kind(f'{what} failed (code {rc}): {msg.decode() if msg else "?"}')


def ptr(t):
    return None if t is None else t.data_ptr()


_raw_stream = getattr(torch._C, '_cuda_getCurrentRawStream', None)


def stream_of(t):
    if _raw_stream is not None:
        idx = t.device.index
        return _raw_stream(idx if idx is not None else torch.cuda.current_device())
    return torch.cuda.current_stream(t.device).cuda_stream


def row_pitch(t):
    if t is None or t.dim() != 4 or t.is_contiguous():
        return 0
    b, c, h, w = t.shape
    sb, sc, sh, sw = t.stride()
    if sw == 1 and sh > w and sc == h * sh and sb == c * sc and sh % 32 == 0 and t.data_ptr() % 16 == 0:
        return sh
    return 0


def require_cuda_f32(*tensors, pitched=()):
    dev = None
    for t in tensors:
        if t is None:
            continue
        if not t.is_cuda:
            raise RuntimeError('gan_control_amd: the HIP hot path needs tensors on a GPU (got %s); there is no CPU fallback' % t.device)
        if t.dtype != torch.float32:
            raise RuntimeError('gan_control_amd: float32 tensors expected, got %s' % t.dtype)
        if not t.is_contiguous() and not (any(t is q for q in pitched) and row_pitch(t)):
            raise RuntimeError('gan_control_amd: internal error: non-contiguous tensor reached the kernel boundary')
        if dev is None:
            dev = t.device
        elif t.device != dev:
            raise RuntimeError('gan_control_amd: tensors on different devices (%s vs %s)' % (dev, t.device))
    return dev
```

### gan-control_amd/gan_control_amd/models/op/conv2d_gradfix.py

```python
import os

import torch
from torch.autograd import Function

from . import _backend
from .upfirdn2d import _dense_or_pitched
from ._backend import ConvGeom
from .weight_layout import adjoint_layout, kernel_layout


_FUSE_PW_ACT = os.environ.get('GANCONTROL_FUSE_PW_ACT', '1') != '0'


def _adjoint_geom(g, in_h, in_w):
    return ConvGeom(g.kh, g.kw, g.down, g.up, g.kh - 1 - g.pad_y, g.kw - 1 - g.pad_x, in_h, in_w)


def _adjoint_weight(w_t):
    return adjoint_layout(w_t)


class _GConv(Function):

    @staticmethod
    def forward(ctx, x, w_t, geom, residual=None):
        ctx.geom = geom
        ctx.in_hw = (x.shape[2], x.shape[3])
        ctx.save_for_backward(x, w_t)
        ctx.set_materialize_grads(False)
        ep = None if residual is None else (None, None, None, 1.0, 1.0, False, residual.contiguous())
        return _backend.get().conv2d(_dense_or_pitched(x), w_t.contiguous(), None, None, geom, epilogue=ep)

    @staticmethod
    def backward(ctx, gy):
        if gy is None:
            return (None,) * len(ctx.needs_input_grad)
        x, w_t = ctx.saved_tensors
        g = ctx.geom
        gx = gw = None
        if ctx.needs_input_grad[0]:
            gx = _backend.call(_GConv, gy, _adjoint_weight(w_t), _adjoint_geom(g, *ctx.in_hw))
        if ctx.needs_input_grad[1] and _backend.want_param_grads():
            gw = _weight_grad(x, gy, g)
        want_res = len(ctx.needs_input_grad) > 3 and ctx.needs_input_grad[3]
        return (gx, gw, None, gy if want_res else None)[:len(ctx.needs_input_grad)]


def _weight_grad(x, gy, g):
    if g.up == 1:
        return _backend.call(_WGrad, x, gy, g)
    swapped = ConvGeom(g.kh, g.kw, 1, g.up, g.kh - 1 - g.pad_y, g.kw - 1 - g.pad_x, x.shape[2], x.shape[3])
    return adjoint_layout(_backend.call(_WGrad, gy, x, swapped))


class _WGrad(Function):
    @staticmethod
    def forward(ctx, x, gy, geom):
        ctx.geom = geom
        ctx.in_hw = (x.shape[2], x.shape[3])
        ctx.save_for_backward(x, gy)
        ctx.set_materialize_grads(False)
        return _backend.get().conv2d_wgrad(_dense_or_pitched(x), _dense_or_pitched(gy), None, None, geom)

    @staticmethod
    def backward(ctx, ggw):
        if ggw is None:
            return None, None, None
        x, gy = ctx.saved_tensors
        g = ctx.geom
        gx = ggy = None
        if ctx.needs_input_grad[0]:
            gx = _backend.call(_GConv, gy, _adjoint_weight(ggw), _adjoint_geom(g, *ctx.in_hw))
        if ctx.needs_input_grad[1]:
            ggy = _backend.call(_GConv, x, ggw.contiguous(), g)
        return gx, ggy, None


class _GConvAct(Function):

    @staticmethod
    def forward(ctx, x, w_t, bias, geom, slope, gain, fork=False, premasked=False):
        out = _backend.get().conv2d(_dense_or_pitched(x), w_t.contiguous(), None, None, geom, epilogue=(bias, None, None, slope, gain, True))
        ctx.geom, ctx.cfg = geom, (slope, gain)
        ctx.premasked = bool(premasked)
        ctx.in_hw = (x.shape[2], x.shape[3])
        ctx.save_for_backward(x, w_t, out)
        ctx.set_materialize_grads(False)
        return (out, x.view_as(x)) if fork else out

    @staticmethod
    def backward(ctx, gy, gfork=None):
        from .fused_act import _BiasActGrad, _BiasActGradReduce
        x, w_t, out = ctx.saved_tensors
        g = ctx.geom
        slope, gain = ctx.cfg
        gx = gw = gb = None
        if not any(ctx.needs_input_grad[:3]):
            return None, None, None, None, None, None, None, None
        if gy is None:
            return (gfork if ctx.needs_input_grad[0] else None), None, None, None, None, None, None, None
        params = _backend.want_param_grads()
        be = _backend.get()
        if (_FUSE_PW_ACT and not ctx.premasked and gfork is None and g.kh == 1 and g.kw == 1 and g.up == 1 and g.down == 1 and g.pad_y == 0
                and not torch.is_grad_enabled() and not _backend.strict_zeros() and getattr(be, 'pw_act_wgrad', None) is not None
                and gy.is_contiguous() and out.is_contiguous() and x.is_contiguous() and be.pw_act_supported(x, gy)):
            if (ctx.needs_input_grad[1] or ctx.needs_input_grad[2]) and params:
                gw_, gb_ = be.pw_act_wgrad(x, gy, out, slope, gain)
                gw = gw_ if ctx.needs_input_grad[1] else None
                gb = gb_ if ctx.needs_input_grad[2] else None
            if ctx.needs_input_grad[0]:
                gx = be.pw_act_dgrad(gy, out, _adjoint_weight(w_t).contiguous(), slope, gain)
            return gx, gw, gb, None, None, None, None, None
        if ctx.premasked:
            from .fused_act import _channel_sum
            g_pre = gy
            if ctx.needs_input_grad[2] and params:
                gb = _channel_sum(gy)
        elif ctx.needs_input_grad[2] and params:
            g_pre, psum = _backend.call(_BiasActGradReduce, gy, out, None, slope, gain)[:2]
            gb = psum.sum((0, 2))
        else:
            g_pre = _backend.call(_BiasActGrad, gy, out, slope, gain)
        if ctx.needs_input_grad[0]:
            gx = _backend.call(_GConv, g_pre, _adjoint_weight(w_t), _adjoint_geom(g, *ctx.in_hw), gfork)
        if ctx.needs_input_grad[1] and params:
            gw = _weight_grad(x, g_pre, g)
        return gx, gw, gb, None, None, None, None, None


def _pair(v):
    return (int(v), int(v)) if not isinstance(v, (tuple, list)) else (int(v[0]), int(v[1]))


def _check(input, weight, stride, padding, dilation, groups):
    if dilation not in (1, (1, 1)) or groups != 1:
        raise ValueError('conv2d_gradfix: only dilation=1, groups=1 are implemented on the HIP path')
    s, p = _pair(stride), _pair(padding)
    if s[0] != s[1] or p[0] != p[1]:
        raise ValueError('conv2d_gradfix: stride and padding must be square')
    if input.ndim != 4 or weight.ndim != 4:
        raise ValueError('conv2d_gradfix: 4-D input and weight expected')
    return s[0], p[0]


def conv2d_t(x, w_t, stride=1, padding=0, residual=None):
    kh, kw = w_t.shape[0], w_t.shape[1]
    oh = (x.shape[2] + 2 * padding - kh) // stride + 1
    ow = (x.shape[3] + 2 * padding - kw) // stride + 1
    return _backend.call(_GConv, x, w_t, ConvGeom(kh, kw, 1, stride, padding, padding, oh, ow), residual)


def conv_transpose2d_t(x, w_t, stride=1, padding=0):
    kh, kw = w_t.shape[0], w_t.shape[1]
    oh = (x.shape[2] - 1) * stride - 2 * padding + kh
    ow = (x.shape[3] - 1) * stride - 2 * padding + kw
    return _backend.call(_GConv, x, w_t, ConvGeom(kh, kw, stride, 1, kh - 1 - padding, kw - 1 - padding, oh, ow))


def conv2d(input, weight, bias=None, stride=1, padding=0, dilation=1, groups=1, weight_scale=1.0, residual=None):
    s, p = _check(input, weight, stride, padding, dilation, groups)
    if weight.shape[1] != input.shape[1]:
        raise ValueError(f'conv2d: weight expects {weight.shape[1]} input channels, got {input.shape[1]}')
    if residual is not None and bias is not None:
        raise NotImplementedError('conv2d: residual together with a plain bias is not built')
    y = conv2d_t(input, kernel_layout(weight, weight_scale), s, p, residual)
    return y if bias is None else y + bias.reshape(1, -1, 1, 1)


def conv2d_bias_act(input, weight, bias, stride=1, padding=0, weight_scale=1.0, negative_slope=0.2, scale=2 ** 0.5, fork=False, grad_premasked=False):
    s, p = _check(input, weight, stride, padding, 1, 1)
    if weight.shape[1] != input.shape[1]:
        raise ValueError(f'conv2d: weight expects {weight.shape[1]} input channels, got {input.shape[1]}')
    if bias.numel() != weight.shape[0]:
        raise ValueError(f'conv2d_bias_act: bias has {bias.numel()} elements, weight has {weight.shape[0]} output channels')
    kh, kw = weight.shape[2], weight.shape[3]
    oh = (input.shape[2] + 2 * p - kh) // s + 1
    ow = (input.shape[3] + 2 * p - kw) // s + 1
    return _backend.call(_GConvAct, input, kernel_layout(weight, weight_scale), bias.reshape(-1).contiguous(),
                           ConvGeom(kh, kw, 1, s, p, p, oh, ow), float(negative_slope), float(scale), bool(fork), bool(grad_premasked))


def conv_transpose2d(input, weight, bias=None, stride=1, padding=0, output_padding=0, groups=1, dilation=1, weight_scale=1.0):
    s, p = _check(input, weight, stride, padding, dilation, groups)
    if output_padding not in (0, (0, 0)):
        raise ValueError('conv_transpose2d: output_padding is not implemented on the HIP path')
    if weight.shape[0] != input.shape[1]:
        raise ValueError(f'conv_transpose2d: weight expects {weight.shape[0]} input channels, got {input.shape[1]}')
    with _backend.pitched_outputs(False):
        y = conv_transpose2d_t(input, kernel_layout(weight, weight_scale, flip=True, in_major=True), s, p)
    return y if bias is None else y + bias.reshape(1, -1, 1, 1)
```

### gan-control_amd/gan_control_amd/models/op/fused_act.py

```python
import torch
from torch import nn
from torch.autograd import Function

from . import _backend


def _channel_sum(t):
    return _backend.call(_ChannelSum, t)


class _ChannelSum(Function):

    @staticmethod
    def forward(ctx, t):
        ctx.shape = t.shape
        ctx.set_materialize_grads(False)
        return _backend.get().channel_sum(t.contiguous())

    @staticmethod
    def backward(ctx, g):
        if g is None:
            return None
        shape = ctx.shape
        return g.reshape([1, -1] + [1] * (len(shape) - 2)).expand(shape)


class _BiasAct(Function):
    @staticmethod
    def forward(ctx, x, bias, noise, noise_w, slope, gain):
        y = _backend.get().bias_act(x.contiguous(), bias, None if noise is None else noise.contiguous(), noise_w, slope, gain)
        ctx.cfg = (slope, gain)
        ctx.has_bias, ctx.has_noise = bias is not None, noise is not None
        ctx.save_for_backward(y, noise if noise is not None else y.new_empty(0), noise_w if noise_w is not None else y.new_empty(0))
        return y

    @staticmethod
    def backward(ctx, gy):
        y, noise, noise_w = ctx.saved_tensors
        slope, gain = ctx.cfg
        gx = gb = gn = gnw = None
        if not any(ctx.needs_input_grad[:4]):
            return None, None, None, None, None, None
        params = _backend.want_param_grads()
        want_b = ctx.has_bias and ctx.needs_input_grad[1] and params
        want_n = ctx.has_noise and ctx.needs_input_grad[2]
        want_nw = ctx.has_noise and ctx.needs_input_grad[3] and params
        if (want_b or want_nw) and not want_n:
            gx, psum, pdot = _backend.call(_BiasActGradReduce, gy, y, noise if want_nw else None, slope, gain)[:3]
            if want_b:
                gb = psum.sum((0, 2))
            if want_nw:
                gnw = pdot.sum().reshape(noise_w.shape)
        else:
            gx = _backend.call(_BiasActGrad, gy, y, slope, gain)
            if want_b:
                gb = _channel_sum(gx)
            if want_n or want_nw:
                per_px = gx.sum(1, keepdim=True)
                if want_n:
                    gn = per_px * noise_w
                if want_nw:
                    gnw = (per_px * noise).sum().reshape(noise_w.shape)
        if not ctx.needs_input_grad[0]:
            gx = None
        return gx, gb, gn, gnw, None, None


REDUCE_CHUNK = 16384


def _spread(partial, like):
    b, c = like.shape[0], like.shape[1]
    inner = like.numel() // (b * c)
    return partial.repeat_interleave(REDUCE_CHUNK, dim=2)[:, :, :inner].reshape(like.shape)


class _BiasActGradReduce(Function):

    @staticmethod
    def forward(ctx, gy, y, noise, slope, gain, bias=None, noise_w=None, self_dot=False):
        ctx.cfg = (slope, gain)
        ctx.has_noise, ctx.self_dot, ctx.has_bias = noise is not None, bool(self_dot), bias is not None
        nz = None if noise is None else noise.contiguous()
        gx, psum, pdot, pself = _backend.get().bias_act_bwd_reduce(gy.contiguous(), y, nz, slope, gain,
                                                                    self_dot=(bias, noise_w if noise is not None else None) if self_dot else None)
        empty = y.new_empty(0)
        ctx.save_for_backward(y, noise if noise is not None else empty, bias if (self_dot and bias is not None) else empty,
                              noise_w if (self_dot and noise is not None) else empty, gx if self_dot else empty)
        dead = []
        if pdot is None:
            pdot = psum.new_empty(0)
            dead.append(pdot)
        if pself is None:
            pself = psum.new_empty(0)
            dead.append(pself)
        if dead:
            ctx.mark_non_differentiable(*dead)
        ctx.set_materialize_grads(False)
        return gx, psum, pdot, pself

    @staticmethod
    def backward(ctx, ggx, gpsum, gpdot, gpself):
        if ggx is None and gpsum is None and gpdot is None and gpself is None:
            return (None,) * 8
        y, noise, bias, noise_w, gx = ctx.saved_tensors
        slope, gain = ctx.cfg
        b = y.shape[0]
        if not torch.is_grad_enabled() and slope != 0 and gain != 0:
            def chunked(t):
                return None if (t is None or t.numel() == 0) else t.contiguous()
            cw = chunked(gpself) if ctx.self_dot else None
            g_gy, g_y, pgb, pgn = _backend.get().bias_act_bwd_reduce_adjoint(
                None if ggx is None else ggx.contiguous(), chunked(gpsum), chunked(gpdot) if ctx.has_noise else None, cw, y,
                gx if cw is not None else None, noise.contiguous() if ctx.has_noise else None, bias if (cw is not None and ctx.has_bias) else None,
                noise_w if (cw is not None and ctx.has_noise) else None, slope, gain, want_gyref=ctx.needs_input_grad[1])
            g_bias = g_nw = None
            if cw is not None and ctx.has_bias and ctx.needs_input_grad[5]:
                g_bias = -pgb.sum((0, 2))
            if cw is not None and ctx.has_noise and ctx.needs_input_grad[6]:
                g_nw = -pgn.sum().reshape(noise_w.shape)
            if g_y is None and ctx.needs_input_grad[1] and _backend.strict_zeros():
                g_y = torch.zeros_like(y)
            return (g_gy if ctx.needs_input_grad[0] else None), g_y, None, None, None, g_bias, g_nw, None
        noise4 = noise.reshape(b, 1, *y.shape[2:]) if ctx.has_noise else None
        total = torch.zeros_like(y) if ggx is None else ggx
        if gpsum is not None:
            total = total + _spread(gpsum, y)
        if ctx.has_noise and gpdot is not None and gpdot.numel() > 0:
            total = total + _spread(gpdot, y) * noise4
        g_y = g_bias = g_nw = None
        if ctx.self_dot and gpself is not None and gpself.numel() > 0:
            w_self = _spread(gpself, y)
            x_pre = torch.where(y > 0, y / gain, y / (gain * slope))
            if ctx.has_bias:
                x_pre = x_pre - bias.reshape([1, -1] + [1] * (y.ndim - 2))
            if ctx.has_noise:
                x_pre = x_pre - noise_w * noise4
            total = total + w_self * x_pre
            wg = w_self * gx
            if ctx.needs_input_grad[1]:
                g_y = torch.where(y > 0, wg / gain, wg / (gain * slope))
            if ctx.has_bias and ctx.needs_input_grad[5]:
                g_bias = -wg.sum([d for d in range(y.ndim) if d != 1])
            if ctx.has_noise and ctx.needs_input_grad[6]:
                g_nw = -(wg * noise4).sum().reshape(noise_w.shape)
        g_gy = _backend.call(_BiasActGrad, total, y, slope, gain) if ctx.needs_input_grad[0] else None
        if g_y is None and ctx.needs_input_grad[1] and _backend.strict_zeros():
            g_y = torch.zeros_like(y)
        return g_gy, g_y, None, None, None, g_bias, g_nw, None


class _BiasActGrad(Function):

    @staticmethod
    def forward(ctx, gy, y, slope, gain):
        ctx.save_for_backward(y)
        ctx.cfg = (slope, gain)
        ctx.set_materialize_grads(False)
        return _backend.get().bias_act_bwd(gy.contiguous(), y, slope, gain)

    @staticmethod
    def backward(ctx, ggx):
        if ggx is None:
            return None, None, None, None
        y, = ctx.saved_tensors
        slope, gain = ctx.cfg
        ggy = _backend.call(_BiasActGrad, ggx, y, slope, gain) if ctx.needs_input_grad[0] else None
        return ggy, (torch.zeros_like(y) if (ctx.needs_input_grad[1] and _backend.strict_zeros()) else None), None, None


def fused_noise_bias_act(input, bias=None, noise=None, noise_weight=None, negative_slope=0.2, scale=2 ** 0.5):
    if (noise is None) != (noise_weight is None):
        raise ValueError('noise and noise_weight go together')
    if bias is not None and bias.numel() != input.shape[1]:
        raise ValueError(f'bias has {bias.numel()} elements, input has {input.shape[1]} channels')
    if bias is not None:
        bias = bias.reshape(-1).contiguous()
    if noise is not None:
        if noise.shape[0] != input.shape[0] or noise.numel() * input.shape[1] != input.numel():
            raise ValueError(f'noise shape {tuple(noise.shape)} does not match input {tuple(input.shape)}')
        noise_weight = noise_weight.reshape(-1).contiguous()
    return _backend.call(_BiasAct, input, bias, noise, noise_weight, float(negative_slope), float(scale))


def fused_leaky_relu(input, bias, negative_slope=0.2, scale=2 ** 0.5):
    return fused_noise_bias_act(input, bias, None, None, negative_slope, scale)


class FusedLeakyReLU(nn.Module):
    def __init__(self, channel, negative_slope=0.2, scale=2 ** 0.5):
        super().__init__()
        self.bias = nn.Parameter(torch.zeros(channel))
        self.negative_slope = negative_slope
        self.scale = scale

    def forward(self, input, noise=None, noise_weight=None):
        return fused_noise_bias_act(input, self.bias, noise, noise_weight, self.negative_slope, self.scale)
```

### gan-control_amd/gan_control_amd/models/op/modulated_conv.py

```python
import math
import os

import torch
from torch.autograd import Function

from . import _backend
from ._backend import ConvGeom
from .conv2d_gradfix import _adjoint_geom, _adjoint_weight
from .weight_layout import kernel_layout
from .upfirdn2d import upfirdn2d, _dense_or_pitched


_WGRAD_SAMPLES = int(os.environ.get('GANCONTROL_WGRAD_SAMPLES', '1'))
_SAMPLES_MIN_RATIO = float(os.environ.get('GANCONTROL_WGRAD_SAMPLES_RATIO', '2'))


def _samples_route(x, gy, g, want_si, want_so, derived=False):
    if not _WGRAD_SAMPLES or torch.is_grad_enabled() or not (want_si or want_so) or (derived and _WGRAD_SAMPLES < 2):
        return False
    be = _backend.get()
    if not hasattr(be, 'conv2d_wgrad_samples_bytes'):
        return False
    saved = 2.0 * ((x.numel() if want_si else 0) + (gy.numel() if want_so else 0))
    extra = 3.0 * x.shape[0] * g.kh * g.kw * x.shape[1] * gy.shape[1]
    if saved < _SAMPLES_MIN_RATIO * extra:
        return False
    if g.up == 1:
        return be.conv2d_wgrad_samples_bytes(_dense_or_pitched(x), gy, g) > 0
    return be.conv2d_wgrad_samples_bytes(_dense_or_pitched(gy), x, _swapped_geom(g, x)) > 0


def _weight_and_scale_grads(x, gy, w_t, si, so, g, want_si, want_so):
    be = _backend.get()
    cs = lambda t: None if t is None else t.contiguous()
    if g.up == 1:
        gw, dws = be.conv2d_wgrad_samples(_dense_or_pitched(x), _dense_or_pitched(gy), cs(si), cs(so), g)
        gsi, gso = be.wgrad_samples_contract(dws, w_t.contiguous(), cs(si), cs(so), want_si, want_so)
        return gw, gsi, gso
    dw_adj, dws = be.conv2d_wgrad_samples(_dense_or_pitched(gy), _dense_or_pitched(x), cs(so), cs(si), _swapped_geom(g, x))
    gso, gsi = be.wgrad_samples_contract(dws, _adjoint_weight(w_t).contiguous(), cs(so), cs(si), want_so, want_si)
    return _adjoint_weight(dw_adj), gsi, gso


def _wsq_value(w):
    run = getattr(_backend.get(), 'weight_prep_batch', None)
    if run is not None and w.is_contiguous():
        return run('wsq', [(w.detach(),)])[0]
    return w.detach().pow(2).sum([2, 3])


class _WeightSq(Function):

    @staticmethod
    def forward(ctx, w):
        from . import weight_cache
        ctx.save_for_backward(w)
        return weight_cache.derive(w, ('wsq',), lambda: _wsq_value(w), recipe=('wsq',)).detach()

    @staticmethod
    def backward(ctx, g):
        w, = ctx.saved_tensors
        return (2.0 * g)[:, :, None, None] * w


class _WeightSqAll(Function):

    _fast = {}

    @staticmethod
    def forward(ctx, *ws):
        from . import weight_cache
        ctx.save_for_backward(*ws)
        key = tuple(id(w._base if w._base is not None else w) for w in ws)
        stamp = (weight_cache.generation[0], tuple(w._version for w in ws), tuple(w.data_ptr() for w in ws))
        hit = _WeightSqAll._fast.get(key)
        if hit is not None and hit[0] == stamp and weight_cache.ENABLED:
            return tuple(t.detach() for t in hit[1])
        outs = [weight_cache.derive(w, ('wsq',), lambda w=w: _wsq_value(w), recipe=('wsq',)) for w in ws]
        stamp = (weight_cache.generation[0], stamp[1], stamp[2])
        if all(weight_cache._derived.get(t.data_ptr()) is not None for t in outs):
            _WeightSqAll._fast[key] = (stamp, outs)
        return tuple(t.detach() for t in outs)

    @staticmethod
    def backward(ctx, *gs):
        ws = ctx.saved_tensors
        be = _backend.get()
        if torch.is_grad_enabled() or getattr(be, 'weight_sq_bwd', None) is None or not all(w.is_contiguous() for w in ws):
            return tuple((2.0 * g)[:, :, None, None] * w if ctx.needs_input_grad[i] else None for i, (g, w) in enumerate(zip(gs, ws)))
        idx = [i for i in range(len(ws)) if ctx.needs_input_grad[i]]
        outs = be.weight_sq_bwd([ws[i] for i in idx], [gs[i].contiguous() for i in idx]) if idx else []
        res = [None] * len(ws)
        for i, o in zip(idx, outs):
            res[i] = o
        return tuple(res)


def weight_sq_all(weights):
    return list(_backend.call(_WeightSqAll, *[w.view(w.shape[-4:]) for w in weights]))


def demod_coefficients(weight, s, scale, eps=1e-8):
    wsq = _backend.call(_WeightSq, weight.view(weight.shape[1:]))
    from .linear import equal_linear
    return torch.rsqrt(equal_linear(s.pow(2), wsq, _eps_vector(s, wsq.shape[0], eps), scale * scale, 1.0))


_EPS_VECTORS = {}


def _eps_vector(like, n, eps):
    key = (like.device, like.dtype, n, eps)
    t = _EPS_VECTORS.get(key)
    if t is None:
        t = _EPS_VECTORS[key] = torch.full((n,), eps, device=like.device, dtype=like.dtype)
    return t


class _SafeDiv(Function):

    @staticmethod
    def forward(ctx, num, den):
        out = _backend.get().rows_sum_div(num.contiguous().unsqueeze(-1), den.contiguous())
        ctx.save_for_backward(den, out)
        ctx.set_materialize_grads(False)
        return out

    @staticmethod
    def backward(ctx, g):
        if g is None:
            return None, None
        den, out = ctx.saved_tensors
        gq = _backend.call(_SafeDiv, g, den)
        return (gq if ctx.needs_input_grad[0] else None), (-(gq * out) if ctx.needs_input_grad[1] else None)


class _SumDiv(Function):

    @staticmethod
    def forward(ctx, partial, den):
        out = _backend.get().rows_sum_div(partial.contiguous(), den.contiguous())
        ctx.save_for_backward(den, out)
        ctx.chunks = partial.shape[-1]
        ctx.set_materialize_grads(False)
        return out

    @staticmethod
    def backward(ctx, g):
        if g is None:
            return None, None
        den, out = ctx.saved_tensors
        gq = _backend.call(_SafeDiv, g, den)
        return (gq.unsqueeze(-1).expand(*gq.shape, ctx.chunks) if ctx.needs_input_grad[0] else None), (-(gq * out) if ctx.needs_input_grad[1] else None)


class _PlaneDot(Function):

    @staticmethod
    def forward(ctx, a, b, den=None):
        out = _backend.get().plane_dot(_dense_or_pitched(a), _dense_or_pitched(b), den)
        ctx.has_den = den is not None
        ctx.save_for_backward(a, b, den if den is not None else a.new_empty(0), out if den is not None else a.new_empty(0))
        ctx.set_materialize_grads(False)
        return out

    @staticmethod
    def backward(ctx, g):
        if g is None:
            return None, None, None
        a, b, den, out = ctx.saved_tensors
        gq = _backend.call(_SafeDiv, g, den) if ctx.has_den else g
        g4 = gq[:, :, None, None]
        return (g4 * b if ctx.needs_input_grad[0] else None), (g4 * a if ctx.needs_input_grad[1] else None), \
            (-(gq * out) if ctx.has_den and ctx.needs_input_grad[2] else None)


class _ModConv(Function):

    @staticmethod
    def forward(ctx, x, w_t, si, so, geom, bias=None, residual=None, fork=False, derived=False):
        ctx.derived = derived
        ep = None
        if bias is not None or residual is not None:
            ep = (bias, None, None, 1.0, 1.0, False, None if residual is None else residual.contiguous())
        y = _backend.get().conv2d(_dense_or_pitched(x), w_t.contiguous(), None if si is None else si.contiguous(),
                                  None if so is None else so.contiguous(), geom, epilogue=ep)
        ctx.geom, ctx.in_hw = geom, (x.shape[2], x.shape[3])
        ctx.has_si, ctx.has_so, ctx.has_bias, ctx.has_res = si is not None, so is not None, bias is not None, residual is not None
        ctx.set_materialize_grads(False)
        empty = x.new_empty(0)
        keep_res = residual if (residual is not None and so is not None) else empty
        keep_bias = bias if (bias is not None and so is not None) else empty
        ctx.save_for_backward(x, w_t, si if si is not None else empty, so if so is not None else empty, y, keep_res, keep_bias)
        return (y, x.view_as(x)) if fork else y

    @staticmethod
    def backward(ctx, gy, gfork=None):
        x, w_t, si, so, y, res, bias = ctx.saved_tensors
        si = si if ctx.has_si else None
        so = so if ctx.has_so else None
        g = ctx.geom
        need = ctx.needs_input_grad
        gx = gw = gsi = gso = gb = gres = None
        if gy is None:
            return (gfork if need[0] else None), None, None, None, None, None, None, None, None
        need_si = ctx.has_si and need[2]
        need_so = ctx.has_so and need[3]
        fused = need[1] and _backend.want_param_grads() and _samples_route(x, gy, g, need_si, need_so, ctx.derived)
        if need[0] or (need_si and not fused):
            gx = _backend.call(_ModConv, gy, _adjoint_weight(w_t), so, si, _adjoint_geom(g, *ctx.in_hw), None, gfork if need[0] else None, False, True)
        if fused:
            gw, gsi, gso = _weight_and_scale_grads(x, gy, w_t, si, so, g, need_si, need_so)
            need_si = need_so = False
        elif need[1] and _backend.want_param_grads():
            gw = _mod_weight_grad(x, gy, si, so, g)
        if need_si:
            conv_part = gx if (gfork is None or not need[0]) else gx - gfork
            gsi = _backend.call(_PlaneDot, x, conv_part, si)
        if need_so:
            conv_part = y
            if ctx.has_res:
                conv_part = conv_part - res
            if ctx.has_bias:
                conv_part = conv_part - bias.reshape(1, -1, 1, 1)
            gso = _backend.call(_PlaneDot, gy, conv_part, so)
        if ctx.has_bias and need[5] and _backend.want_param_grads():
            from .fused_act import _channel_sum
            gb = _channel_sum(gy)
        if ctx.has_res and need[6]:
            gres = gy
        return (gx if need[0] else None), gw, gsi, gso, None, gb, gres, None, None


class _ModConvAct(Function):

    @staticmethod
    def forward(ctx, x, w_t, si, so, bias, noise, noise_w, geom, slope, gain):
        out = _backend.get().conv2d(x.contiguous(), w_t.contiguous(), None if si is None else si.contiguous(),
                                    None if so is None else so.contiguous(), geom,
                                    epilogue=(bias, None if noise is None else noise.contiguous(), noise_w, slope, gain, True))
        ctx.geom, ctx.in_hw, ctx.cfg = geom, (x.shape[2], x.shape[3]), (slope, gain)
        ctx.has = (si is not None, so is not None, bias is not None, noise is not None)
        empty = x.new_empty(0)
        ctx.save_for_backward(x, w_t, *[t if t is not None else empty for t in (si, so, bias, noise, noise_w)], out)
        ctx.set_materialize_grads(False)
        return out

    @staticmethod
    def backward(ctx, gy):
        from .fused_act import _BiasActGrad, _BiasActGradReduce
        x, w_t, si, so, bias, noise, noise_w, out = ctx.saved_tensors
        has_si, has_so, has_bias, has_noise = ctx.has
        si, so, bias = (si if has_si else None), (so if has_so else None), (bias if has_bias else None)
        noise, noise_w = (noise, noise_w) if has_noise else (None, None)
        g, (slope, gain) = ctx.geom, ctx.cfg
        need = ctx.needs_input_grad
        gx = gw = gsi = gso = gb = gnw = None
        if gy is None or not any(need[:7]):
            return (None,) * 10
        want_so = has_so and need[3]
        if not _backend.want_param_grads():
            need = list(need)
            need[1] = need[4] = need[6] = False
        if (has_bias and need[4]) or (has_noise and need[6]) or want_so:
            g_pre, psum, pdot, pself = _backend.call(_BiasActGradReduce, gy, out, noise, slope, gain, bias, noise_w, want_so)
            if has_bias and need[4]:
                gb = psum.sum((0, 2))
            if has_noise and need[6]:
                gnw = pdot.sum().reshape(noise_w.shape)
            if want_so:
                gso = _backend.call(_SumDiv, pself, so)
        else:
            g_pre = _backend.call(_BiasActGrad, gy, out, slope, gain)
        need_si = has_si and need[2]
        fused = need[1] and _samples_route(x, g_pre, g, need_si, False)
        if need[0] or (need_si and not fused):
            gx = _backend.call(_ModConv, g_pre, _adjoint_weight(w_t), so, si, _adjoint_geom(g, *ctx.in_hw), None, None, False, True)
        if fused:
            gw, gsi, _ = _weight_and_scale_grads(x, g_pre, w_t, si, so, g, True, False)
        elif need[1]:
            gw = _mod_weight_grad(x, g_pre, si, so, g)
        if need_si and not fused:
            gsi = _backend.call(_PlaneDot, x, gx, si)
        return (gx if need[0] else None), gw, gsi, gso, gb, None, gnw, None, None, None


def _swapped_geom(g, x):
    return ConvGeom(g.kh, g.kw, 1, g.up, g.kh - 1 - g.pad_y, g.kw - 1 - g.pad_x, x.shape[2], x.shape[3])


def _mod_weight_grad(x, gy, si, so, g):
    if g.up == 1:
        return _backend.call(_ModWGrad, x, gy, si, so, g)
    return _adjoint_weight(_backend.call(_ModWGrad, gy, x, so, si, _swapped_geom(g, x)))


class _ModWGrad(Function):

    @staticmethod
    def forward(ctx, x, gy, si, so, geom):
        ctx.geom, ctx.in_hw = geom, (x.shape[2], x.shape[3])
        ctx.has_si, ctx.has_so = si is not None, so is not None
        empty = x.new_empty(0)
        ctx.save_for_backward(x, gy, si if si is not None else empty, so if so is not None else empty)
        ctx.set_materialize_grads(False)
        return _backend.get().conv2d_wgrad(_dense_or_pitched(x), _dense_or_pitched(gy), None if si is None else si.contiguous(),
                                           None if so is None else so.contiguous(), geom)

    @staticmethod
    def backward(ctx, ggw):
        if ggw is None:
            return None, None, None, None, None
        x, gy, si, so = ctx.saved_tensors
        si = si if ctx.has_si else None
        so = so if ctx.has_so else None
        g = ctx.geom
        gx = ggy = gsi = gso = None
        need_si = ctx.has_si and ctx.needs_input_grad[2]
        need_so = ctx.has_so and ctx.needs_input_grad[3]
        if ctx.needs_input_grad[0] or need_si:
            gx = _backend.call(_ModConv, gy, _adjoint_weight(ggw), so, si, _adjoint_geom(g, *ctx.in_hw), None, None, False, True)
        if ctx.needs_input_grad[1] or need_so:
            ggy = _backend.call(_ModConv, x, ggw.contiguous(), si, so, g, None, None, False, True)
        if need_si:
            gsi = _backend.call(_PlaneDot, x, gx, si)
        if need_so:
            gso = _backend.call(_PlaneDot, gy, ggy, so)
        return (gx if ctx.needs_input_grad[0] else None), (ggy if ctx.needs_input_grad[1] else None), gsi, gso, None


def modulated_conv2d(x, weight, s, demodulate=True, upsample=False, blur_kernel=None, blur_pad=None, padding=None, apply_blur=True,
                     bias=None, residual=None, fork=False, demod=None):
    _, oc, ic, k, _ = weight.shape
    scale = 1.0 / math.sqrt(ic * k * k)
    d = (demod if demod is not None else demod_coefficients(weight, s, scale)) if demodulate else None
    if upsample:
        if bias is not None or residual is not None or fork:
            raise NotImplementedError('modulated_conv2d: bias / residual / fork are built for the plain branch only')
        w_t = kernel_layout(weight.view(oc, ic, k, k), scale, flip=True)
        oh, ow = (x.shape[2] - 1) * 2 + k, (x.shape[3] - 1) * 2 + k
        y = _backend.call(_ModConv, x, w_t, s, d, ConvGeom(k, k, 2, 1, k - 1, k - 1, oh, ow))
        return upfirdn2d(y, blur_kernel, pad=blur_pad) if apply_blur else y
    pad = k // 2 if padding is None else padding
    w_t = kernel_layout(weight.view(oc, ic, k, k), scale)
    oh, ow = x.shape[2] + 2 * pad - k + 1, x.shape[3] + 2 * pad - k + 1
    if bias is None and residual is None and not fork:
        return _backend.call(_ModConv, x, w_t, s, d, ConvGeom(k, k, 1, 1, pad, pad, oh, ow))
    return _backend.call(_ModConv, x, w_t, s, d, ConvGeom(k, k, 1, 1, pad, pad, oh, ow), None if bias is None else bias.reshape(-1).contiguous(), residual, bool(fork))


def modulated_conv2d_act(x, weight, s, bias, noise, noise_weight, demodulate=True, padding=None, negative_slope=0.2, act_scale=2 ** 0.5, demod=None):
    _, oc, ic, k, _ = weight.shape
    scale = 1.0 / math.sqrt(ic * k * k)
    d = (demod if demod is not None else demod_coefficients(weight, s, scale)) if demodulate else None
    pad = k // 2 if padding is None else padding
    w_t = kernel_layout(weight.view(oc, ic, k, k), scale)
    oh, ow = x.shape[2] + 2 * pad - k + 1, x.shape[3] + 2 * pad - k + 1
    if noise.shape[0] != x.shape[0] or noise.numel() != x.shape[0] * oh * ow:
        raise ValueError(f'noise shape {tuple(noise.shape)} does not match the output [{x.shape[0]}, {oc}, {oh}, {ow}]')
    return _backend.call(_ModConvAct, x, w_t, s, d, bias.reshape(-1).contiguous(), noise, noise_weight.reshape(-1).contiguous(),
                             ConvGeom(k, k, 1, 1, pad, pad, oh, ow), float(negative_slope), float(act_scale))
```

### gan-control_amd/gan_control_amd/models/op/upfirdn2d.py

```python
import torch
from torch.autograd import Function

import os

from . import _backend

_FUSE_ACT_BWD = os.environ.get('GANCONTROL_FUSE_ACT_BWD_BLUR', '1') != '0'


def _out_size(n, k, up, down, p0, p1):
    return (n * up + p0 + p1 - k) // down + 1


def _dense_or_pitched(x):
    from ... import _lib
    return x if (x.is_cuda and _lib.row_pitch(x)) else x.contiguous()


class _UpFirDn2d(Function):
    @staticmethod
    def forward(ctx, x, kernel, up, down, p0, p1):
        kh, kw = kernel.shape
        n, c, h, w = x.shape
        oh, ow = _out_size(h, kh, up, down, p0, p1), _out_size(w, kw, up, down, p0, p1)
        if oh < 1 or ow < 1:
            raise ValueError(f'upfirdn2d: empty output for input {h}x{w}, kernel {kh}x{kw}, up={up}, down={down}, pad=({p0},{p1})')
        ctx.save_for_backward(kernel)
        ctx.cfg = (up, down, p0, p1, h, w)
        ctx.set_materialize_grads(False)
        return _backend.get().upfirdn2d(_dense_or_pitched(x), kernel, up, down, p0, p0, oh, ow, True)

    @staticmethod
    def backward(ctx, gy):
        kernel, = ctx.saved_tensors
        gx = _backend.call(_UpFirDn2dAdjoint, gy, kernel, ctx.cfg) if (ctx.needs_input_grad[0] and gy is not None) else None
        return gx, None, None, None, None, None


class _UpFirDn2dAdjoint(Function):

    @staticmethod
    def forward(ctx, gy, kernel, cfg):
        up, down, p0, p1, h, w = cfg
        kh, kw = kernel.shape
        ctx.save_for_backward(kernel)
        ctx.cfg = cfg
        ctx.set_materialize_grads(False)
        return _backend.get().upfirdn2d(_dense_or_pitched(gy), kernel, down, up, kw - 1 - p0, kh - 1 - p0, h, w, False)

    @staticmethod
    def backward(ctx, ggx):
        kernel, = ctx.saved_tensors
        up, down, p0, p1, h, w = ctx.cfg
        ggy = _backend.call(_UpFirDn2d, ggx, kernel, up, down, p0, p1) if (ctx.needs_input_grad[0] and ggx is not None) else None
        return ggy, None, None


def upfirdn2d(input, kernel, up=1, down=1, pad=(0, 0), _internal=False):
    if _internal:
        return _backend.call(_UpFirDn2d, input, kernel, int(up), int(down), int(pad[0]), int(pad[1]))
    with _backend.pitched_outputs(False):
        return _backend.call(_UpFirDn2d, input, kernel, int(up), int(down), int(pad[0]), int(pad[1]))


class _BlurOfActivation(Function):

    @staticmethod
    def forward(ctx, a, kernel, p0, p1, slope, gain):
        kh, kw = kernel.shape
        n, c, h, w = a.shape
        oh, ow = _out_size(h, kh, 1, 1, p0, p1), _out_size(w, kw, 1, 1, p0, p1)
        ctx.save_for_backward(kernel, a)
        ctx.cfg, ctx.act = (1, 1, p0, p1, h, w), (slope, gain)
        ctx.set_materialize_grads(False)
        return _backend.get().upfirdn2d(_dense_or_pitched(a), kernel, 1, 1, p0, p0, oh, ow, True)

    @staticmethod
    def backward(ctx, gy):
        kernel, a = ctx.saved_tensors
        if gy is None or not ctx.needs_input_grad[0]:
            return None, None, None, None, None, None
        return _backend.call(_BlurAdjointMasked, gy, kernel, ctx.cfg, a, *ctx.act), None, None, None, None, None


class _BlurAdjointMasked(Function):

    @staticmethod
    def forward(ctx, gy, kernel, cfg, a, slope, gain):
        up, down, p0, p1, h, w = cfg
        kh, kw = kernel.shape
        ctx.save_for_backward(kernel, a)
        ctx.cfg, ctx.act = cfg, (slope, gain)
        ctx.set_materialize_grads(False)
        be = _backend.get()
        fused = getattr(be, 'upfirdn2d_mask', None)
        if (fused is not None and not _backend.strict_zeros() and a.is_contiguous()
                and be.upfirdn2d_act_supported(kernel, 1, 1, h, w, a.shape[0] * a.shape[1])):
            return fused(_dense_or_pitched(gy), kernel, kw - 1 - p0, kh - 1 - p0, h, w, False, a, slope, gain)
        g = be.upfirdn2d(_dense_or_pitched(gy), kernel, down, up, kw - 1 - p0, kh - 1 - p0, h, w, False)
        return be.bias_act_bwd(g.contiguous(), a.contiguous(), slope, gain)

    @staticmethod
    def backward(ctx, gg):
        from .fused_act import _BiasActGrad
        kernel, a = ctx.saved_tensors
        if gg is None:
            return None, None, None, None, None, None
        up, down, p0, p1, h, w = ctx.cfg
        slope, gain = ctx.act
        ggy = _backend.call(_UpFirDn2d, _backend.call(_BiasActGrad, gg, a, slope, gain), kernel, up, down, p0, p1) if ctx.needs_input_grad[0] else None
        ga = torch.zeros_like(a) if (ctx.needs_input_grad[3] and _backend.strict_zeros()) else None
        return ggy, None, None, ga, None, None


def blur_of_activation(a, kernel, pad, negative_slope, scale):
    return _backend.call(_BlurOfActivation, a, kernel, int(pad[0]), int(pad[1]), float(negative_slope), float(scale))


class _UpFirDn2dAct(Function):

    @staticmethod
    def forward(ctx, x, kernel, p0, p1, bias, noise, noise_w, slope, gain):
        kh, kw = kernel.shape
        n, c, h, w = x.shape
        oh, ow = _out_size(h, kh, 1, 1, p0, p1), _out_size(w, kw, 1, 1, p0, p1)
        out = _backend.get().upfirdn2d_act(_dense_or_pitched(x), kernel, p0, p0, oh, ow, True, bias, None if noise is None else noise.contiguous(), noise_w, slope, gain)
        ctx.cfg, ctx.act = (1, 1, p0, p1, h, w), (slope, gain)
        ctx.has_bias, ctx.has_noise = bias is not None, noise is not None
        empty = x.new_empty(0)
        ctx.save_for_backward(kernel, out, noise if noise is not None else empty, noise_w if noise_w is not None else empty)
        ctx.set_materialize_grads(False)
        return out

    @staticmethod
    def backward(ctx, gy):
        from .fused_act import _BiasActGrad, _BiasActGradReduce
        kernel, out, noise, noise_w = ctx.saved_tensors
        slope, gain = ctx.act
        need = ctx.needs_input_grad
        gx = gb = gnw = None
        params = _backend.want_param_grads()
        want_b, want_nw = ctx.has_bias and need[4] and params, ctx.has_noise and need[6] and params
        if gy is None or not (need[0] or want_b or want_nw):
            return (None,) * 9
        be = _backend.get()
        up, down, p0, p1, h, w = ctx.cfg
        kh, kw = kernel.shape
        fused = getattr(be, 'upfirdn2d_actbwd', None)
        if (fused is not None and _FUSE_ACT_BWD and need[0] and not torch.is_grad_enabled() and not _backend.strict_zeros()
                and gy.is_contiguous() and out.is_contiguous() and 0 <= p0 <= min(kh, kw) - 1
                and be.upfirdn2d_act_supported(kernel, 1, 1, h, w, gy.shape[0] * gy.shape[1])):
            gx, psum, pdot = fused(gy, out, noise.contiguous() if want_nw else None, kernel, kw - 1 - p0, kh - 1 - p0, h, w, False, slope, gain)
            if want_b:
                gb = psum.sum((0, 2))
            if want_nw:
                gnw = pdot.sum().reshape(noise_w.shape)
            return gx, None, None, None, gb, None, gnw, None, None
        if want_b or want_nw:
            g_pre, psum, pdot = _backend.call(_BiasActGradReduce, gy, out, noise if want_nw else None, slope, gain)[:3]
            if want_b:
                gb = psum.sum((0, 2))
            if want_nw:
                gnw = pdot.sum().reshape(noise_w.shape)
        else:
            g_pre = _backend.call(_BiasActGrad, gy, out, slope, gain)
        if need[0]:
            gx = _backend.call(_UpFirDn2dAdjoint, g_pre, kernel, ctx.cfg)
        return gx, None, None, None, gb, None, gnw, None, None


def upfirdn2d_bias_act(input, kernel, pad, bias, noise=None, noise_weight=None, negative_slope=0.2, scale=2 ** 0.5):
    from .fused_act import fused_noise_bias_act
    p0, p1 = int(pad[0]), int(pad[1])
    kh, kw = kernel.shape
    oh, ow = _out_size(input.shape[2], kh, 1, 1, p0, p1), _out_size(input.shape[3], kw, 1, 1, p0, p1)
    if oh >= 1 and ow >= 1 and _backend.get().upfirdn2d_act_supported(kernel, 1, 1, oh, ow, input.shape[0] * input.shape[1]):
        if (noise is None) != (noise_weight is None):
            raise ValueError('noise and noise_weight go together')
        if noise is not None and (noise.shape[0] != input.shape[0] or noise.numel() != input.shape[0] * oh * ow):
            raise ValueError(f'noise shape {tuple(noise.shape)} does not match the output [{input.shape[0]}, {input.shape[1]}, {oh}, {ow}]')
        return _backend.call(_UpFirDn2dAct, input, kernel, p0, p1, None if bias is None else bias.reshape(-1).contiguous(), noise,
                                   None if noise_weight is None else noise_weight.reshape(-1).contiguous(), float(negative_slope), float(scale))
    return fused_noise_bias_act(upfirdn2d(input, kernel, pad=pad), bias, noise, noise_weight, negative_slope, scale)
```

### include/gancontrol_hip.h

```cpp
#ifndef GANCONTROL_HIP_H
#define GANCONTROL_HIP_H

#include <stddef.h>
#include <stdint.h>

#ifdef __cplusplus
extern "C" {
#endif

#define GC_ABI_VERSION 2

#define GC_OK 0
#define GC_ERR_BAD_ARG (-1)
#define GC_ERR_UNSUPPORTED (-2)
#define GC_ERR_HIP (-3)
#define GC_ERR_WORKSPACE (-4)

typedef void* gc_stream_t;

int gc_abi_version(void);
const char* gc_last_error(void);
#define GC_STRUCT_COUNT 6
int gc_struct_sizes(size_t* sizes, int n);
const char* gc_source_hash(void);

int gc_upfirdn2d_f32(const float* x, const float* taps, float* y,
                     int planes, int in_h, int in_w, int out_h, int out_w,
                     int kh, int kw, int up_x, int up_y, int down_x, int down_y,
                     int pad_x0, int pad_y0, int flip_taps, gc_stream_t stream);

int gc_upfirdn2d_pitched_f32(const float* x, const float* taps, float* y, int batch, int channels, int in_h, int in_w, int in_pitch,
                             int out_h, int out_w, int out_pitch, int kh, int kw, int pad_x0, int pad_y0, int flip_taps, int activate,
                             const float* bias, const float* noise, const float* noise_w, float slope, float gain, gc_stream_t stream);

int gc_upfirdn2d_act_f32(const float* x, const float* taps, float* y,
                         int batch, int channels, int in_h, int in_w, int out_h, int out_w,
                         int kh, int kw, int pad_x0, int pad_y0, int flip_taps,
                         const float* bias, const float* noise, const float* noise_w, float slope, float gain,
                         gc_stream_t stream);

int gc_upfirdn2d_mask_f32(const float* x, const float* taps, float* y, int batch, int channels, int in_h, int in_w, int in_pitch,
                          int out_h, int out_w, int kh, int kw, int pad_x0, int pad_y0, int flip_taps,
                          const float* mask_ref, float slope, float gain, gc_stream_t stream);

int gc_upfirdn2d_actbwd_tiles(int out_h, int out_w);
int gc_upfirdn2d_actbwd_f32(const float* gy, const float* y_ref, const float* noise, const float* taps, float* gx, float* psum, float* pdot,
                            int batch, int channels, int in_h, int in_w, int out_h, int out_w, int out_pitch, int kh, int kw,
                            int pad_x0, int pad_y0, int flip_taps, float slope, float gain, gc_stream_t stream);

int gc_bias_act_f32(const float* x, const float* bias, const float* noise, const float* noise_w,
                    float* y, int batch, int channels, int64_t inner,
                    float slope, float gain, gc_stream_t stream);

int gc_bias_act_bwd_f32(const float* dy, const float* y_ref, float* dx, int64_t count,
                        float slope, float gain, gc_stream_t stream);

int gc_bias_act_bwd_chunks(int64_t inner);
int gc_bias_act_bwd_reduce_f32(const float* dy, const float* y_ref, const float* noise, float* dx,
                               float* psum, float* pdot, int batch, int channels, int64_t inner,
                               float slope, float gain, gc_stream_t stream);

int gc_bias_act_bwd_reduce_self_f32(const float* dy, const float* y_ref, const float* noise, const float* bias, const float* noise_w,
                                    float* dx, float* psum, float* pdot, float* pself, int batch, int channels, int64_t inner,
                                    float slope, float gain, gc_stream_t stream);

int gc_bias_act_bwd_reduce_adjoint_f32(const float* ggx, const float* cs, const float* cd, const float* cw, const float* y_ref, const float* dx,
                                       const float* noise, const float* bias, const float* noise_w, float* g_dy, float* g_yref, float* pgb, float* pgn,
                                       int batch, int channels, int64_t inner, float slope, float gain, gc_stream_t stream);

int gc_plane_dot_f32(const float* a, const float* b, float* partial, int planes, int64_t inner, gc_stream_t stream);

int gc_plane_dot_pitched_chunks(int rows);
int gc_plane_dot_pitched_f32(const float* a, const float* b, float* partial, int planes, int rows, int width, int a_pitch, int b_pitch, gc_stream_t stream);

int gc_rows_sum_div_f32(const float* partial, const float* den, float* out, int rows, int chunks, gc_stream_t stream);

size_t gc_channel_sum_workspace(int batch, int channels, int64_t inner);
int gc_channel_sum_f32(const float* x, float* out, int batch, int channels, int64_t inner,
                       void* workspace, size_t workspace_bytes, gc_stream_t stream);

typedef struct gc_conv_desc {
    int32_t batch;
    int32_t in_ch, out_ch;
    int32_t in_h, in_w;
    int32_t out_h, out_w;
    int32_t kh, kw;
    int32_t up, down;
    int32_t pad_y, pad_x;
    int32_t in_pitch;
    int32_t out_pitch;
} gc_conv_desc;

int gc_small_gemm_ok(int M, int K, int N, int64_t sb0, int64_t sb1);
int gc_small_gemm_f32(const float* a, int64_t sa0, int64_t sa1, const float* b, int64_t sb0, int64_t sb1,
                      const float* bias, float beta, float alpha, float* out, int M, int K, int N, gc_stream_t stream);

int gc_conv2d_out_pitch(const gc_conv_desc* d, int mode);

int gc_conv2d_in_pitch_ok(const gc_conv_desc* d, int mode, int wgrad);

int gc_conv2d_f32(const gc_conv_desc* d, const float* x, const float* w,
                  const float* in_scale, const float* out_scale, float* y, gc_stream_t stream);

typedef struct gc_conv_epilogue {
    const float* bias;
    const float* noise;
    const float* noise_w;
    float slope, gain;
    int32_t activate;
    const float* residual;
} gc_conv_epilogue;

int gc_conv2d_fused_f32(const gc_conv_desc* d, const float* x, const float* w,
                        const float* in_scale, const float* out_scale, const gc_conv_epilogue* ep,
                        float* y, gc_stream_t stream);

size_t gc_conv2d_f32_workspace(const gc_conv_desc* d);
int gc_conv2d_fused_f32_ws(const gc_conv_desc* d, const float* x, const float* w,
                           const float* in_scale, const float* out_scale, const gc_conv_epilogue* ep,
                           float* y, void* workspace, size_t workspace_bytes, gc_stream_t stream);

size_t gc_conv2d_bf16x3_workspace(const gc_conv_desc* d);
int gc_conv2d_bf16x3_f32(const gc_conv_desc* d, const float* x, const float* w,
                         const float* in_scale, const float* out_scale, float* y,
                         void* workspace, size_t workspace_bytes, gc_stream_t stream);

int gc_conv2d_fused_bf16x3_f32(const gc_conv_desc* d, const float* x, const float* w,
                               const float* in_scale, const float* out_scale, const gc_conv_epilogue* ep, float* y,
                               void* workspace, size_t workspace_bytes, gc_stream_t stream);

size_t gc_conv2d_bf16x3_packed_bytes(const gc_conv_desc* d);
size_t gc_conv2d_bf16x3_splitk_bytes(const gc_conv_desc* d);
int gc_conv2d_pack_weights_bf16x3(const gc_conv_desc* d, const float* w, void* packed, size_t packed_bytes, gc_stream_t stream);
int gc_conv2d_fused_bf16x3_packed_f32(const gc_conv_desc* d, const float* x, const float* w, const void* packed, size_t packed_bytes,
                                      const float* in_scale, const float* out_scale, const gc_conv_epilogue* ep, float* y,
                                      void* workspace, size_t workspace_bytes, gc_stream_t stream);

int gc_conv2d_fused_bf16_packed_f32(const gc_conv_desc* d, const float* x, const float* w, const void* packed, size_t packed_bytes,
                                    const float* in_scale, const float* out_scale, const gc_conv_epilogue* ep, float* y,
                                    void* workspace, size_t workspace_bytes, gc_stream_t stream);

int gc_conv2d_variant_name(const gc_conv_desc* d, int mode, char* name, int name_bytes);

size_t gc_conv2d_wgrad_workspace(const gc_conv_desc* d);
int gc_conv2d_wgrad_f32(const gc_conv_desc* d, const float* x, const float* dy,
                        const float* in_scale, const float* out_scale, float* dw,
                        void* workspace, size_t workspace_bytes, gc_stream_t stream);

size_t gc_conv2d_wgrad_bf16x3_workspace(const gc_conv_desc* d);
int gc_conv2d_wgrad_bf16x3_f32(const gc_conv_desc* d, const float* x, const float* dy,
                               const float* in_scale, const float* out_scale, float* dw,
                               void* workspace, size_t workspace_bytes, gc_stream_t stream);

int gc_conv2d_wgrad_bf16_f32(const gc_conv_desc* d, const float* x, const float* dy,
                             const float* in_scale, const float* out_scale, float* dw,
                             void* workspace, size_t workspace_bytes, gc_stream_t stream);

int gc_conv2d_wgrad_variant_name(const gc_conv_desc* d, int mode, int samples, char* name, int name_bytes);

size_t gc_conv2d_wgrad_samples_workspace(const gc_conv_desc* d, int mode);
int gc_conv2d_wgrad_samples_f32(const gc_conv_desc* d, const float* x, const float* dy, const float* in_scale, const float* out_scale,
                                float* dw, float* dw_samples, void* workspace, size_t workspace_bytes, gc_stream_t stream);
int gc_conv2d_wgrad_samples_bf16x3_f32(const gc_conv_desc* d, const float* x, const float* dy, const float* in_scale, const float* out_scale,
                                       float* dw, float* dw_samples, void* workspace, size_t workspace_bytes, gc_stream_t stream);
int gc_conv2d_wgrad_samples_bf16_f32(const gc_conv_desc* d, const float* x, const float* dy, const float* in_scale, const float* out_scale,
                                     float* dw, float* dw_samples, void* workspace, size_t workspace_bytes, gc_stream_t stream);

size_t gc_wgrad_samples_contract_workspace(int batch, int a, int c);
int gc_wgrad_samples_contract_f32(const float* dw_samples, const float* w, const float* scale_a, const float* scale_c, float* g_a, float* g_c,
                                  int batch, int taps, int a, int c, void* workspace, size_t workspace_bytes, gc_stream_t stream);

int gc_weight_layout_f32(const float* src, float* dst, int taps, int k, int n,
                         const int64_t src_stride[3], const int64_t dst_stride[3],
                         int flip_taps, float scale, gc_stream_t stream);

int gc_affine_warp_bilinear_f32(const float* x, const float* mat, float* y, int batch, int channels,
                                int in_h, int in_w, int out_h, int out_w, int adjoint, gc_stream_t stream);
int gc_reflect_pad_f32(const float* x, float* y, int planes, int in_h, int in_w, int left, int right, int top, int bottom,
                       int adjoint, gc_stream_t stream);

typedef struct gc_wlayout_group {
    const float* src;
    float* dst;
    int32_t taps, k, n, flip_taps;
    int64_t src_stride[3], dst_stride[3];
    float scale;
} gc_wlayout_group;
int gc_weight_layout_grouped_f32(const gc_wlayout_group* groups, int n_groups, gc_stream_t stream);

typedef struct gc_wpack_group {
    gc_conv_desc desc;
    const float* w;
    void* packed;
    size_t packed_bytes;
} gc_wpack_group;
int gc_conv2d_pack_weights_bf16x3_grouped(const gc_wpack_group* groups, int n_groups, gc_stream_t stream);

size_t gc_pw_act_wgrad_workspace(int batch, int k, int n, int64_t plane);
int gc_pw_act_wgrad_f32(const float* x, const float* dy, const float* y_ref, float* dw_db, int batch, int k, int n, int64_t plane,
                        float slope, float gain, void* workspace, size_t workspace_bytes, gc_stream_t stream);
int gc_pw_act_dgrad_f32(const float* dy, const float* y_ref, const float* w, float* gx, int batch, int n, int k, int64_t plane,
                        float slope, float gain, gc_stream_t stream);

typedef struct gc_glin_group {
    float* x;
    float* w;
    float* bias;
    float* y;
    int32_t n, k;
    int64_t x_stride;
    float alpha, beta;
} gc_glin_group;
int gc_grouped_linear_f32(const gc_glin_group* groups, int n_groups, int batch, gc_stream_t stream);
int gc_grouped_linear_bwd_x_f32(const gc_glin_group* groups, int n_groups, int batch, gc_stream_t stream);
int gc_grouped_linear_bwd_w_f32(const gc_glin_group* groups, int n_groups, int batch, gc_stream_t stream);

typedef struct gc_wsq_group {
    const float* w;
    const float* g;
    float* out;
    int32_t rows, taps;
} gc_wsq_group;
int gc_weight_sq_grouped_f32(const gc_wsq_group* groups, int n_groups, gc_stream_t stream);
int gc_weight_sq_bwd_grouped_f32(const gc_wsq_group* groups, int n_groups, gc_stream_t stream);


int gc_conv2d_bn_relu_f32(const float* x, const float* w, const float* scale, const float* shift, float* y,
                          int batch, int in_ch, int out_ch, int in_h, int in_w, int kh, int kw, int stride, int pad_y, int pad_x,
                          int relu, int out_channels, int chan_off, gc_stream_t stream);

int gc_pool2d_f32(const float* x, float* y, int batch, int channels, int in_h, int in_w, int k, int stride, int pad, int mode,
                  int out_channels, int chan_off, gc_stream_t stream);

int gc_global_avgpool_f32(const float* x, float* y, int planes, int inner, gc_stream_t stream);

int gc_resize_bilinear_f32(const float* x, float* y, int planes, int in_h, int in_w, int out_h, int out_w, float mul, float add, gc_stream_t stream);


int gc_crop_resize_ac_f32(const float* x, float* y, int planes, int in_h, int in_w, int top, int left, int crop_h, int crop_w,
                          int out_h, int out_w, int adjoint, gc_stream_t stream);

int gc_affine_prelu_f32(const float* x, const float* scale, const float* shift, const float* alpha, float* y, int batch, int channels,
                        int hw, gc_stream_t stream);

int gc_affine_prelu_bwd_f32(const float* g, const float* x, const float* scale, const float* shift, const float* alpha, const float* g2,
                            int g2_mode, float* gx, int batch, int channels, int h, int w, gc_stream_t stream);

int gc_plane_reduce_f32(const float* a, const float* b, float* out, int planes, int inner, float mul, gc_stream_t stream);

int gc_se_mlp_f32(const float* m, const float* fc1, const float* fc2, float* z, float* s, int batch, int channels, int red, gc_stream_t stream);

int gc_se_mlp_bwd_f32(const float* t, const float* s, const float* z, const float* fc1, const float* fc2, float* gm, int batch, int channels,
                      int red, float mul, gc_stream_t stream);

int gc_se_apply_f32(const float* r, const float* s, const float* sc, float* out, int planes, int h, int w, int sc_h, int sc_w, int sc_stride,
                    gc_stream_t stream);

int gc_image_u8_to_f32(const uint8_t* x, int64_t row_stride, int64_t sample_stride, const float* lut, const int32_t* flip, float* y,
                       int batch, int h, int w, gc_stream_t stream);
int gc_image_resample_u8(const uint8_t* x, int64_t row_stride, int64_t sample_stride, int in_h, int in_w, uint8_t* y, int batch,
                         int out_h, int out_w, int axis, const int32_t* coeff, const int32_t* bounds, const int32_t* bounds_host,
                         int kmax, int table_stride, const int32_t* other, const int32_t* other_host, gc_stream_t stream);
int gc_image_resample_v_u8_to_f32(const uint8_t* x, int64_t row_stride, int64_t sample_stride, int in_h, int in_w, const float* lut,
                                  const int32_t* flip, float* y, int batch, int out_h, int out_w, const int32_t* coeff,
                                  const int32_t* bounds, const int32_t* bounds_host, int kmax, int table_stride, const int32_t* other,
                                  const int32_t* other_host, gc_stream_t stream);

int gc_image_f32_to_u8_grid(const float* x, int64_t row_stride, int64_t plane_stride, int64_t sample_stride, uint8_t* y, int64_t y_row_stride,
                            int batch, int h, int w, int nrow, int padding, int pad_value, int grid_h, int grid_w, gc_stream_t stream);

#ifdef __cplusplus
}
#endif
#endif
```

Before: 81.52 images/sec.

## Fuse backward bias/noise/style partial reductions into single finish kernels and blur sums

Adds a combined finish kernel that reduces bias-sum, noise-dot and style-row partials in one launch instead of several torch sum ops and a separate sum-div launch. Adds a single-pass wave-per-plane dot kernel for small planes, and makes the blur-mask backward kernel also emit per-tile output sums. These sums are handed to the next bias-act backward through a pointer/version-checked slot. The aim is to cut launch count and small-reduction overhead in the backward passes, at the cost of extra code paths and a global handoff state that could go stale if the checks miss a case.

```diff
diff --git a/gan-control_amd/csrc/bias_act.hip b/gan-control_amd/csrc/bias_act.hip
--- a/gan-control_amd/csrc/bias_act.hip
+++ b/gan-control_amd/csrc/bias_act.hip
@@ -225,6 +225,74 @@
     out[r] = acc;
 }
 
+__device__ __forceinline__ float wave_sum_all(float v) {
+#pragma unroll
+    for (int off = 32; off > 0; off >>= 1) v += __shfl_xor(v, off, 64);
+    return v;
+}
+
+__global__ __launch_bounds__(256) void plane_dot_small_kernel(const float* __restrict__ a, const float* __restrict__ b, const float* __restrict__ den,
+                                                              float* __restrict__ out, int planes, int inner) {
+    const int lane = threadIdx.x & 63, plane = blockIdx.x * 4 + (threadIdx.x >> 6);
+    if (plane >= planes) return;
+    const float* ap = a + (size_t)plane * inner;
+    const float* bp = b + (size_t)plane * inner;
+    typedef float f4u __attribute__((ext_vector_type(4), aligned(4)));
+    const int n4 = inner >> 2;
+    float acc = 0.f;
+#pragma unroll 4
+    for (int v = lane; v < n4; v += 64) {
+        const f4u a4 = *reinterpret_cast<const f4u*>(ap + 4 * v), b4 = *reinterpret_cast<const f4u*>(bp + 4 * v);
+        acc = fmaf(a4.x, b4.x, acc); acc = fmaf(a4.y, b4.y, acc); acc = fmaf(a4.z, b4.z, acc); acc = fmaf(a4.w, b4.w, acc);
+    }
+    for (int i = 4 * n4 + lane; i < inner; i += 64) acc = fmaf(ap[i], bp[i], acc);
+    acc = wave_sum_all(acc);
+    if (lane == 0) {
+        if (den) { const float d = den[plane]; acc = acc / (d == 0.f ? 1.f : d); }
+        out[plane] = acc;
+    }
+}
+
+__global__ __launch_bounds__(256) void bias_act_partials_finish_kernel(
+    const float* __restrict__ psum, float* __restrict__ gb, const float* __restrict__ pdot, float* __restrict__ dot,
+    const float* __restrict__ pself, const float* __restrict__ den, float* __restrict__ rows,
+    int batch, int channels, int chunks, int64_t dot_count, float sign, int gb_blocks, int dot_blocks) {
+    __shared__ float lds[4];
+    const int lane = threadIdx.x & 63, wave = threadIdx.x >> 6;
+    int blk = blockIdx.x;
+    if (blk < gb_blocks) {
+        const int c = blk * 4 + wave;
+        if (c >= channels) return;
+        const int n = batch * chunks;
+        float acc = 0.f;
+        for (int i = lane; i < n; i += 64) {
+            const int bi = i / chunks, j = i - bi * chunks;
+            acc += psum[((size_t)bi * channels + c) * chunks + j];
+        }
+        acc = wave_sum_all(acc);
+        if (lane == 0) gb[c] = sign * acc;
+        return;
+    }
+    blk -= gb_blocks;
+    if (blk < dot_blocks) {
+        float acc = 0.f;
+        for (int64_t i = threadIdx.x; i < dot_count; i += 256) acc += pdot[i];
+        const float r = block_sum(acc, lds);
+        if (threadIdx.x == 0) dot[0] = sign * r;
+        return;
+    }
+    blk -= dot_blocks;
+    const int r = blk * 4 + wave;
+    if (r >= batch * channels) return;
+    float acc = 0.f;
+    for (int j = lane; j < chunks; j += 64) acc += pself[(size_t)r * chunks + j];
+    acc = wave_sum_all(acc);
+    if (lane == 0) {
+        if (den) { const float d = den[r]; acc = acc / (d == 0.f ? 1.f : d); }
+        rows[r] = acc;
+    }
+}
+
 __global__ __launch_bounds__(256) void plane_dot_pitched_kernel(const float* __restrict__ a, const float* __restrict__ b, float* __restrict__ partial,
                                                                 int rows, int width, int a_pitch, int b_pitch, int chunks, int rpc) {
     __shared__ float lds[4];
@@ -465,3 +533,28 @@
     hipLaunchKernelGGL(plane_dot_kernel, dim3((unsigned)chunks * (unsigned)planes), dim3(256), 0, (hipStream_t)stream, a, b, partial, inner, chunks, len);
     return gc::check_launch("gc_plane_dot_f32");
 }
+
+extern "C" int gc_plane_dot_small_f32(const float* a, const float* b, const float* den, float* out, int planes, int64_t inner, gc_stream_t stream) {
+    if (!a || !b || !out) return gc::fail(GC_ERR_BAD_ARG, "gc_plane_dot_small_f32: null pointer");
+    if (planes <= 0 || inner <= 0) return gc::fail(GC_ERR_BAD_ARG, "gc_plane_dot_small_f32: bad extents");
+    if (gc_bias_act_bwd_chunks(inner) != 1) return gc::fail(GC_ERR_UNSUPPORTED, "gc_plane_dot_small_f32: planes of one chunk only (inner = %lld)", (long long)inner);
+    hipLaunchKernelGGL(plane_dot_small_kernel, dim3((unsigned)gc::ceil_div(planes, 4)), dim3(256), 0, (hipStream_t)stream, a, b, den, out, planes, (int)inner);
+    return gc::check_launch("gc_plane_dot_small_f32");
+}
+
+extern "C" int gc_partials_finish_f32(const float* psum, float* gb, const float* pdot, float* dot, const float* pself, const float* den, float* rows,
+                                      int batch, int channels, int chunks, int64_t dot_count, float sign, gc_stream_t stream) {
+    if ((psum == nullptr) != (gb == nullptr) || (pdot == nullptr) != (dot == nullptr) || (pself == nullptr) != (rows == nullptr))
+        return gc::fail(GC_ERR_BAD_ARG, "gc_partials_finish_f32: every input goes with its output");
+    if (den && !pself) return gc::fail(GC_ERR_BAD_ARG, "gc_partials_finish_f32: den without pself");
+    if (!psum && !pdot && !pself) return GC_OK;
+    if ((psum || pself) && (batch <= 0 || channels <= 0 || chunks <= 0)) return gc::fail(GC_ERR_BAD_ARG, "gc_partials_finish_f32: bad extents");
+    if (pdot && dot_count <= 0) return gc::fail(GC_ERR_BAD_ARG, "gc_partials_finish_f32: bad dot_count");
+    if ((psum || pself) && (int64_t)batch * channels > INT32_MAX - 4) return gc::fail(GC_ERR_UNSUPPORTED, "gc_partials_finish_f32: more than 2^31 rows");
+    if ((psum || pself) && (int64_t)batch * chunks > INT32_MAX) return gc::fail(GC_ERR_UNSUPPORTED, "gc_partials_finish_f32: more than 2^31 partial sums per channel");
+    const int gb_blocks = psum ? gc::ceil_div(channels, 4) : 0, dot_blocks = pdot ? 1 : 0;
+    const int row_blocks = pself ? gc::ceil_div(batch * channels, 4) : 0;
+    hipLaunchKernelGGL(bias_act_partials_finish_kernel, dim3((unsigned)(gb_blocks + dot_blocks + row_blocks)), dim3(256), 0, (hipStream_t)stream,
+                       psum, gb, pdot, dot, pself, den, rows, batch, channels, chunks, dot_count, sign, gb_blocks, dot_blocks);
+    return gc::check_launch("gc_partials_finish_f32");
+}
diff --git a/gan-control_amd/csrc/upfirdn2d.hip b/gan-control_amd/csrc/upfirdn2d.hip
--- a/gan-control_amd/csrc/upfirdn2d.hip
+++ b/gan-control_amd/csrc/upfirdn2d.hip
@@ -25,7 +25,7 @@
 #else
 #define GC_FIR_BOUNDS __launch_bounds__(256)
 #endif
-template <bool VEC, int EPI, bool PRO = false>
+template <bool VEC, int EPI, bool PRO = false, bool SUMS = false>
 __global__ GC_FIR_BOUNDS void fir44_tile_kernel(
     const float* __restrict__ x, const float* __restrict__ taps, float* __restrict__ y,
     int in_h, int in_w, int out_h, int out_w, int pad_x0, int pad_y0, int flip, FirEpilogue ep, int in_pitch, int out_pitch) {
@@ -62,6 +62,7 @@
         return v;
     };
     static_assert(!PRO || GC_FIR_NT == 1, "the prologue sums are written once per workgroup");
+    static_assert(!SUMS || (EPI == 2 && !PRO && GC_FIR_NT == 1), "the output sums belong to the mask epilogue and are written once per workgroup");
     float ps = 0.f, pd = 0.f;
     const float* refp = PRO ? ep.pro_ref + plane * (size_t)in_h * in_w : nullptr;
     const float* nzp = (PRO && ep.pro_noise) ? ep.pro_noise + (plane / ep.channels) * (size_t)in_h * in_w : nullptr;
@@ -165,6 +166,24 @@
             for (int r = 0; r < 4; ++r)
 #pragma unroll
                 for (int j = 0; j < 4; ++j) acc[r][j] *= m[r][j] > 0.f ? ep.mpos : ep.mneg;
+        }
+        if (SUMS) {
+            float os = 0.f;
+#pragma unroll
+            for (int r = 0; r < 4; ++r) {
+                const bool row_in = oy0 + rg * 4 + r < out_h;
+                const float s0 = (row_in && ox < out_w) ? acc[r][0] : 0.f, s1 = (row_in && ox + 1 < out_w) ? acc[r][1] : 0.f;
+                const float s2 = (row_in && ox + 2 < out_w) ? acc[r][2] : 0.f, s3 = (row_in && ox + 3 < out_w) ? acc[r][3] : 0.f;
+                os += (s0 + s1) + (s2 + s3);
+            }
+#pragma unroll
+            for (int off = 32; off > 0; off >>= 1) os += __shfl_xor(os, off, 64);
+            if ((tid & 63) == 0) red[tid >> 6] = os;
+            __syncthreads();
+            if (tid == 0) {
+                const size_t slot = plane * ((size_t)gridDim.x * gridDim.y) + (size_t)blockIdx.y * gridDim.x + blockIdx.x;
+                ep.pro_psum[slot] = (red[0] + red[1]) + (red[2] + red[3]);
+            }
         }
         if (EPI == 1) {
             const int c = (int)(plane % ep.channels);
@@ -550,8 +569,9 @@
     if (out_h <= 0 || out_w <= 0) return gc::fail(GC_ERR_BAD_ARG, "gc_upfirdn2d_f32: empty output (%d x %d)", out_h, out_w);
     if (planes == 0) return GC_OK;
     hipStream_t s = (hipStream_t)stream;
+    const bool sums = ep && ep->mask_ref && ep->pro_psum;
     const bool fast = up_x == 1 && up_y == 1 && down_x == 1 && down_y == 1 && kh == 4 && kw == 4 &&
-                      out_w >= 64 && out_h >= 16 && planes <= 65535;
+                      ((out_w >= 64 && out_h >= 16) || sums) && planes <= 65535;
     if (ep && !fast) return gc::fail(GC_ERR_UNSUPPORTED, "gc_upfirdn2d_act_f32: the fused epilogue needs the 4x4, up = down = 1 tile kernel (planes >= 64 x 16)");
     if ((in_pitch != in_w || out_pitch != out_w) && !fast) return gc::fail(GC_ERR_UNSUPPORTED, "gc_upfirdn2d_pitched_f32: a pitched input needs the 4x4, up = down = 1 tile kernel (planes >= 64 x 16)");
     if (fast) {
@@ -564,6 +584,11 @@
             else     hipLaunchKernelGGL((fir44_tile_kernel<false, 0, true>), grid, dim3(256), 0, s, x, taps, y, in_h, in_w, out_h, out_w, pad_x0, pad_y0, flip_taps, *ep, in_pitch, out_pitch);
             return gc::check_launch("gc_upfirdn2d_actbwd_f32");
         }
+        if (sums) {
+            if (vec) hipLaunchKernelGGL((fir44_tile_kernel<true, 2, false, true>), grid, dim3(256), 0, s, x, taps, y, in_h, in_w, out_h, out_w, pad_x0, pad_y0, flip_taps, *ep, in_pitch, out_pitch);
+            else     hipLaunchKernelGGL((fir44_tile_kernel<false, 2, false, true>), grid, dim3(256), 0, s, x, taps, y, in_h, in_w, out_h, out_w, pad_x0, pad_y0, flip_taps, *ep, in_pitch, out_pitch);
+            return gc::check_launch("gc_upfirdn2d_mask_sums_f32");
+        }
 #define GC_FIR(V, E) hipLaunchKernelGGL((fir44_tile_kernel<V, E>), grid, dim3(256), 0, s, x, taps, y, in_h, in_w, out_h, out_w, pad_x0, pad_y0, flip_taps, ep ? *ep : none, in_pitch, out_pitch)
         if (ep && ep->mask_ref) { if (vec) GC_FIR(true, 2); else GC_FIR(false, 2); }
         else if (ep) { if (vec) GC_FIR(true, 1); else GC_FIR(false, 1); }
@@ -652,6 +677,21 @@
     return upfirdn2d_impl(x, taps, y, batch * channels, in_h, in_w, out_h, out_w, kh, kw, 1, 1, 1, 1, pad_x0, pad_y0, flip_taps, &ep, stream, in_pitch, 0);
 }
 
+extern "C" int gc_upfirdn2d_mask_sums_tiles(int out_h, int out_w) {
+    return gc_upfirdn2d_actbwd_tiles(out_h, out_w);
+}
+
+extern "C" int gc_upfirdn2d_mask_sums_f32(const float* x, const float* taps, float* y, float* psum, int batch, int channels, int in_h, int in_w, int in_pitch,
+                                          int out_h, int out_w, int kh, int kw, int pad_x0, int pad_y0, int flip_taps,
+                                          const float* mask_ref, float slope, float gain, gc_stream_t stream) {
+    if (!mask_ref || !psum) return gc::fail(GC_ERR_BAD_ARG, "gc_upfirdn2d_mask_sums_f32: null pointer");
+    if (batch < 0 || channels <= 0) return gc::fail(GC_ERR_BAD_ARG, "gc_upfirdn2d_mask_sums_f32: bad batch / channels");
+    if (kh != 4 || kw != 4 || (int64_t)batch * channels > 65535)
+        return gc::fail(GC_ERR_UNSUPPORTED, "gc_upfirdn2d_mask_sums_f32: needs 4 x 4 taps and at most 65535 planes");
+    const FirEpilogue ep{nullptr, nullptr, nullptr, 1.f, 1.f, channels, mask_ref, gain, gain * slope, nullptr, nullptr, psum, nullptr, 1.f, 1.f};
+    return upfirdn2d_impl(x, taps, y, batch * channels, in_h, in_w, out_h, out_w, kh, kw, 1, 1, 1, 1, pad_x0, pad_y0, flip_taps, &ep, stream, in_pitch, 0);
+}
+
 extern "C" int gc_upfirdn2d_act_f32(const float* x, const float* taps, float* y,
                                     int batch, int channels, int in_h, int in_w, int out_h, int out_w,
                                     int kh, int kw, int pad_x0, int pad_y0, int flip_taps,
diff --git a/gan-control_amd/gan_control_amd/_lib.py b/gan-control_amd/gan_control_amd/_lib.py
--- a/gan-control_amd/gan_control_amd/_lib.py
+++ b/gan-control_amd/gan_control_amd/_lib.py
@@ -81,6 +81,10 @@
     'gc_upfirdn2d_actbwd_tiles': (_i32, [_i32, _i32]),
     'gc_upfirdn2d_actbwd_f32': (_i32, [_vp] * 7 + [_i32] * 12 + [_f32, _f32, _vp]),
     'gc_upfirdn2d_mask_f32': (_i32, [_vp, _vp, _vp] + [_i32] * 12 + [_vp, _f32, _f32, _vp]),
+    'gc_upfirdn2d_mask_sums_tiles': (_i32, [_i32, _i32]),
+    'gc_upfirdn2d_mask_sums_f32': (_i32, [_vp, _vp, _vp, _vp] + [_i32] * 12 + [_vp, _f32, _f32, _vp]),
+    'gc_plane_dot_small_f32': (_i32, [_vp, _vp, _vp, _vp, _i32, _i64, _vp]),
+    'gc_partials_finish_f32': (_i32, [_vp] * 7 + [_i32, _i32, _i32, _i64, _f32, _vp]),
     'gc_upfirdn2d_pitched_f32': (_i32, [_vp, _vp, _vp] + [_i32] * 14 + [_vp, _vp, _vp, _f32, _f32, _vp]),
     'gc_plane_dot_pitched_chunks': (_i32, [_i32]),
     'gc_plane_dot_pitched_f32': (_i32, [_vp, _vp, _vp, _i32, _i32, _i32, _i32, _i32, _vp]),
diff --git a/gan-control_amd/gan_control_amd/models/op/_backward_sums.py b/gan-control_amd/gan_control_amd/models/op/_backward_sums.py
--- /dev/null
+++ b/gan-control_amd/gan_control_amd/models/op/_backward_sums.py
@@ -0,0 +1,110 @@
+import torch
+
+from ... import _lib
+from . import _backend
+
+
+def _hip():
+    be = _backend.get()
+    return be if getattr(be, 'name', None) == 'hip' else None
+
+
+def available():
+    return _hip() is not None
+
+
+def plain_backward():
+    return not torch.is_grad_enabled() and not _backend.strict_zeros()
+
+
+
+_SLOT = [None]
+
+
+def offer(g_pre, psum):
+    _SLOT[0] = (g_pre, g_pre.data_ptr(), tuple(g_pre.shape), g_pre._version, psum)
+
+
+def clear():
+    _SLOT[0] = None
+
+
+def take(gy):
+    held, _SLOT[0] = _SLOT[0], None
+    if held is None or gy is None:
+        return None
+    _, ptr, shape, version, psum = held
+    if gy.data_ptr() != ptr or tuple(gy.shape) != shape or gy._version != version or not gy.is_contiguous():
+        return None
+    return psum
+
+
+
+def upfirdn2d_mask_sums(x, taps, pad_x0, pad_y0, out_h, out_w, flip, mask_ref, slope, gain):
+    be = _hip()
+    if be is None:
+        return None
+    pitch = _lib.row_pitch(x)
+    dev = _lib.require_cuda_f32(x, taps, mask_ref, pitched=(x,))
+    n, c, h, w = x.shape
+    if tuple(mask_ref.shape) != (n, c, out_h, out_w):
+        raise RuntimeError('upfirdn2d_mask_sums: mask reference %s, output [%d, %d, %d, %d]' % (tuple(mask_ref.shape), n, c, out_h, out_w))
+    if n * c == 0 or tuple(taps.shape) != (4, 4) or n * c > 65535:
+        return None
+    tiles = _lib.load().gc_upfirdn2d_mask_sums_tiles(out_h, out_w)
+    y = _backend.torch.empty((n, c, out_h, out_w), dtype=x.dtype, device=dev)
+    psum = _backend.torch.empty((n, c, tiles), dtype=x.dtype, device=dev)
+    be._launch(dev, 'gc_upfirdn2d_mask_sums_f32', _lib.ptr(x), _lib.ptr(taps), _lib.ptr(y), _lib.ptr(psum), n, c, h, w, pitch or w, out_h, out_w,
+               taps.shape[0], taps.shape[1], pad_x0, pad_y0, int(flip), _lib.ptr(mask_ref), float(slope), float(gain), _lib.stream_of(x),
+               timed=be.timer and (lambda: ('fir44', 'fir44_tile_kernel', 4.0 * (x.numel() + 2 * y.numel()))))
+    return y, psum
+
+
+def finish(psum=None, pdot=None, pself=None, den=None, sign=1.0):
+    be = _hip()
+    if be is None:
+        return None
+    groups = [t for t in (psum, pdot, pself) if t is not None]
+    if not groups or any(t.numel() == 0 for t in groups):
+        return None
+    dev = _lib.require_cuda_f32(psum, pdot, pself, den)
+    shaped = [t for t in (psum, pself) if t is not None]
+    if any(t.dim() != 3 for t in shaped) or len({tuple(t.shape) for t in shaped}) > 1:
+        raise RuntimeError('finish: psum / pself must be [B, C, J] of one shape, got %s' % [tuple(t.shape) for t in shaped])
+    b, c, j = shaped[0].shape if shaped else (1, 1, 1)
+    if den is not None and (pself is None or den.numel() != b * c):
+        raise RuntimeError('finish: den goes with pself and holds B * C elements')
+    gb = _backend.torch.empty(c, dtype=torch.float32, device=dev) if psum is not None else None
+    dot = _backend.torch.empty(1, dtype=torch.float32, device=dev) if pdot is not None else None
+    rows = _backend.torch.empty((b, c), dtype=torch.float32, device=dev) if pself is not None else None
+    be._launch(dev, 'gc_partials_finish_f32', _lib.ptr(psum), _lib.ptr(gb), _lib.ptr(pdot), _lib.ptr(dot), _lib.ptr(pself), _lib.ptr(den), _lib.ptr(rows),
+               b, c, j, 0 if pdot is None else pdot.numel(), float(sign), _lib.stream_of(groups[0]))
+    return gb, dot, rows
+
+
+def bias_noise_grads(psum, pdot, want_b, want_nw, noise_w, sign=1.0):
+    if not (want_b or want_nw):
+        return None, None
+    done = finish(psum if want_b else None, pdot if want_nw else None, sign=sign) if plain_backward() else None
+    if done is not None:
+        return done[0], (done[1].reshape(noise_w.shape) if want_nw else None)
+    gb = psum.sum((0, 2)) if want_b else None
+    gnw = pdot.sum().reshape(noise_w.shape) if want_nw else None
+    if sign < 0:
+        gb, gnw = (None if gb is None else -gb), (None if gnw is None else -gnw)
+    return gb, gnw
+
+
+def plane_dot_small(a, b, den=None):
+    be = _hip()
+    if be is None or a.dim() < 2 or not (a.is_contiguous() and b.is_contiguous()) or a.numel() == 0 or a.shape != b.shape:
+        return None
+    batch, ch = a.shape[0], a.shape[1]
+    inner = a.numel() // (batch * ch)
+    if be._bwd_chunks(inner) != 1:
+        return None
+    den = None if den is None else den.contiguous()
+    dev = _lib.require_cuda_f32(a, b, den)
+    out = _backend.torch.empty((batch, ch), dtype=a.dtype, device=dev)
+    be._launch(dev, 'gc_plane_dot_small_f32', _lib.ptr(a), _lib.ptr(b), _lib.ptr(den), _lib.ptr(out), batch * ch, inner, _lib.stream_of(a))
+    return out
diff --git a/gan-control_amd/gan_control_amd/models/op/conv2d_gradfix.py b/gan-control_amd/gan_control_amd/models/op/conv2d_gradfix.py
--- a/gan-control_amd/gan_control_amd/models/op/conv2d_gradfix.py
+++ b/gan-control_amd/gan_control_amd/models/op/conv2d_gradfix.py
@@ -3,7 +3,7 @@
 import torch
 from torch.autograd import Function
 
-from . import _backend
+from . import _backend, _backward_sums
 from .upfirdn2d import _dense_or_pitched
 from ._backend import ConvGeom
 from .weight_layout import adjoint_layout, kernel_layout
@@ -114,11 +114,13 @@
         if ctx.premasked:
             from .fused_act import _channel_sum
             g_pre = gy
+            psum = _backward_sums.take(gy)
             if ctx.needs_input_grad[2] and params:
-                gb = _channel_sum(gy)
+                done = _backward_sums.finish(psum) if (psum is not None and _backward_sums.plain_backward()) else None
+                gb = done[0] if done is not None else _channel_sum(gy)
         elif ctx.needs_input_grad[2] and params:
             g_pre, psum = _backend.call(_BiasActGradReduce, gy, out, None, slope, gain)[:2]
-            gb = psum.sum((0, 2))
+            gb = _backward_sums.bias_noise_grads(psum, None, True, False, None)[0]
         else:
             g_pre = _backend.call(_BiasActGrad, gy, out, slope, gain)
         if ctx.needs_input_grad[0]:
diff --git a/gan-control_amd/gan_control_amd/models/op/fused_act.py b/gan-control_amd/gan_control_amd/models/op/fused_act.py
--- a/gan-control_amd/gan_control_amd/models/op/fused_act.py
+++ b/gan-control_amd/gan_control_amd/models/op/fused_act.py
@@ -2,7 +2,7 @@
 from torch import nn
 from torch.autograd import Function
 
-from . import _backend
+from . import _backend, _backward_sums
 
 
 def _channel_sum(t):
@@ -47,10 +47,7 @@
         want_nw = ctx.has_noise and ctx.needs_input_grad[3] and params
         if (want_b or want_nw) and not want_n:
             gx, psum, pdot = _backend.call(_BiasActGradReduce, gy, y, noise if want_nw else None, slope, gain)[:3]
-            if want_b:
-                gb = psum.sum((0, 2))
-            if want_nw:
-                gnw = pdot.sum().reshape(noise_w.shape)
+            gb, gnw = _backward_sums.bias_noise_grads(psum, pdot, want_b, want_nw, noise_w)
         else:
             gx = _backend.call(_BiasActGrad, gy, y, slope, gain)
             if want_b:
@@ -114,11 +111,8 @@
                 None if ggx is None else ggx.contiguous(), chunked(gpsum), chunked(gpdot) if ctx.has_noise else None, cw, y,
                 gx if cw is not None else None, noise.contiguous() if ctx.has_noise else None, bias if (cw is not None and ctx.has_bias) else None,
                 noise_w if (cw is not None and ctx.has_noise) else None, slope, gain, want_gyref=ctx.needs_input_grad[1])
-            g_bias = g_nw = None
-            if cw is not None and ctx.has_bias and ctx.needs_input_grad[5]:
-                g_bias = -pgb.sum((0, 2))
-            if cw is not None and ctx.has_noise and ctx.needs_input_grad[6]:
-                g_nw = -pgn.sum().reshape(noise_w.shape)
+            g_bias, g_nw = _backward_sums.bias_noise_grads(pgb, pgn, cw is not None and ctx.has_bias and ctx.needs_input_grad[5],
+                                                           cw is not None and ctx.has_noise and ctx.needs_input_grad[6], noise_w, sign=-1.0)
             if g_y is None and ctx.needs_input_grad[1] and _backend.strict_zeros():
                 g_y = torch.zeros_like(y)
             return (g_gy if ctx.needs_input_grad[0] else None), g_y, None, None, None, g_bias, g_nw, None
diff --git a/gan-control_amd/gan_control_amd/models/op/modulated_conv.py b/gan-control_amd/gan_control_amd/models/op/modulated_conv.py
--- a/gan-control_amd/gan_control_amd/models/op/modulated_conv.py
+++ b/gan-control_amd/gan_control_amd/models/op/modulated_conv.py
@@ -4,7 +4,7 @@
 import torch
 from torch.autograd import Function
 
-from . import _backend
+from . import _backend, _backward_sums
 from ._backend import ConvGeom
 from .conv2d_gradfix import _adjoint_geom, _adjoint_weight
 from .weight_layout import kernel_layout
@@ -158,7 +158,10 @@
 
     @staticmethod
     def forward(ctx, a, b, den=None):
-        out = _backend.get().plane_dot(_dense_or_pitched(a), _dense_or_pitched(b), den)
+        a_, b_ = _dense_or_pitched(a), _dense_or_pitched(b)
+        out = None if _backend.strict_zeros() else _backward_sums.plane_dot_small(a_, b_, den)
+        if out is None:
+            out = _backend.get().plane_dot(a_, b_, den)
         ctx.has_den = den is not None
         ctx.save_for_backward(a, b, den if den is not None else a.new_empty(0), out if den is not None else a.new_empty(0))
         ctx.set_materialize_grads(False)
@@ -264,12 +267,15 @@
             need[1] = need[4] = need[6] = False
         if (has_bias and need[4]) or (has_noise and need[6]) or want_so:
             g_pre, psum, pdot, pself = _backend.call(_BiasActGradReduce, gy, out, noise, slope, gain, bias, noise_w, want_so)
-            if has_bias and need[4]:
-                gb = psum.sum((0, 2))
-            if has_noise and need[6]:
-                gnw = pdot.sum().reshape(noise_w.shape)
-            if want_so:
-                gso = _backend.call(_SumDiv, pself, so)
+            want_b, want_nw = bool(has_bias and need[4]), bool(has_noise and need[6])
+            done = _backward_sums.finish(psum if want_b else None, pdot if want_nw else None, pself if want_so else None,
+                                         so.contiguous() if want_so else None) if _backward_sums.plain_backward() else None
+            if done is not None:
+                gb, gnw, gso = done[0], (done[1].reshape(noise_w.shape) if want_nw else None), done[2]
+            else:
+                gb, gnw = _backward_sums.bias_noise_grads(psum, pdot, want_b, want_nw, noise_w)
+                if want_so:
+                    gso = _backend.call(_SumDiv, pself, so)
         else:
             g_pre = _backend.call(_BiasActGrad, gy, out, slope, gain)
         need_si = has_si and need[2]
diff --git a/gan-control_amd/gan_control_amd/models/op/upfirdn2d.py b/gan-control_amd/gan_control_amd/models/op/upfirdn2d.py
--- a/gan-control_amd/gan_control_amd/models/op/upfirdn2d.py
+++ b/gan-control_amd/gan_control_amd/models/op/upfirdn2d.py
@@ -3,7 +3,7 @@
 
 import os
 
-from . import _backend
+from . import _backend, _backward_sums
 
 _FUSE_ACT_BWD = os.environ.get('GANCONTROL_FUSE_ACT_BWD_BLUR', '1') != '0'
 
@@ -94,8 +94,14 @@
         ctx.set_materialize_grads(False)
         be = _backend.get()
         fused = getattr(be, 'upfirdn2d_mask', None)
+        _backward_sums.clear()
         if (fused is not None and not _backend.strict_zeros() and a.is_contiguous()
                 and be.upfirdn2d_act_supported(kernel, 1, 1, h, w, a.shape[0] * a.shape[1])):
+            if _backend.want_param_grads():
+                both = _backward_sums.upfirdn2d_mask_sums(_dense_or_pitched(gy), kernel, kw - 1 - p0, kh - 1 - p0, h, w, False, a, slope, gain)
+                if both is not None:
+                    _backward_sums.offer(*both)
+                    return both[0]
             return fused(_dense_or_pitched(gy), kernel, kw - 1 - p0, kh - 1 - p0, h, w, False, a, slope, gain)
         g = be.upfirdn2d(_dense_or_pitched(gy), kernel, down, up, kw - 1 - p0, kh - 1 - p0, h, w, False)
         return be.bias_act_bwd(g.contiguous(), a.contiguous(), slope, gain)
@@ -151,17 +157,11 @@
                 and gy.is_contiguous() and out.is_contiguous() and 0 <= p0 <= min(kh, kw) - 1
                 and be.upfirdn2d_act_supported(kernel, 1, 1, h, w, gy.shape[0] * gy.shape[1])):
             gx, psum, pdot = fused(gy, out, noise.contiguous() if want_nw else None, kernel, kw - 1 - p0, kh - 1 - p0, h, w, False, slope, gain)
-            if want_b:
-                gb = psum.sum((0, 2))
-            if want_nw:
-                gnw = pdot.sum().reshape(noise_w.shape)
+            gb, gnw = _backward_sums.bias_noise_grads(psum, pdot, want_b, want_nw, noise_w)
             return gx, None, None, None, gb, None, gnw, None, None
         if want_b or want_nw:
             g_pre, psum, pdot = _backend.call(_BiasActGradReduce, gy, out, noise if want_nw else None, slope, gain)[:3]
-            if want_b:
-                gb = psum.sum((0, 2))
-            if want_nw:
-                gnw = pdot.sum().reshape(noise_w.shape)
+            gb, gnw = _backward_sums.bias_noise_grads(psum, pdot, want_b, want_nw, noise_w)
         else:
             g_pre = _backend.call(_BiasActGrad, gy, out, slope, gain)
         if need[0]:
diff --git a/include/gancontrol_hip.h b/include/gancontrol_hip.h
--- a/include/gancontrol_hip.h
+++ b/include/gancontrol_hip.h
@@ -43,6 +43,11 @@
                           int out_h, int out_w, int kh, int kw, int pad_x0, int pad_y0, int flip_taps,
                           const float* mask_ref, float slope, float gain, gc_stream_t stream);
 
+int gc_upfirdn2d_mask_sums_tiles(int out_h, int out_w);
+int gc_upfirdn2d_mask_sums_f32(const float* x, const float* taps, float* y, float* psum, int batch, int channels, int in_h, int in_w, int in_pitch,
+                               int out_h, int out_w, int kh, int kw, int pad_x0, int pad_y0, int flip_taps,
+                               const float* mask_ref, float slope, float gain, gc_stream_t stream);
+
 int gc_upfirdn2d_actbwd_tiles(int out_h, int out_w);
 int gc_upfirdn2d_actbwd_f32(const float* gy, const float* y_ref, const float* noise, const float* taps, float* gx, float* psum, float* pdot,
                             int batch, int channels, int in_h, int in_w, int out_h, int out_w, int out_pitch, int kh, int kw,
@@ -74,6 +79,11 @@
 int gc_plane_dot_pitched_f32(const float* a, const float* b, float* partial, int planes, int rows, int width, int a_pitch, int b_pitch, gc_stream_t stream);
 
 int gc_rows_sum_div_f32(const float* partial, const float* den, float* out, int rows, int chunks, gc_stream_t stream);
+
+int gc_plane_dot_small_f32(const float* a, const float* b, const float* den, float* out, int planes, int64_t inner, gc_stream_t stream);
+
+int gc_partials_finish_f32(const float* psum, float* gb, const float* pdot, float* dot, const float* pself, const float* den, float* rows,
+                           int batch, int channels, int chunks, int64_t dot_count, float sign, gc_stream_t stream);
 
 size_t gc_channel_sum_workspace(int batch, int channels, int64_t inner);
 int gc_channel_sum_f32(const float* x, float* out, int batch, int channels, int64_t inner,
```

Result: no change. 82.27 images/sec, median of 3 (+0.9%).
